# yanconglin/ICP-Flow

Hardware: AMD Instinct MI355X
Metric: cluster-pair ICP registrations/sec (higher is better)
Workload: dtype f32

## Files before the change

### icp_flow_amd/_lib.py

```python
import contextlib
import ctypes
import os
import threading

import torch

_HERE = os.path.dirname(os.path.abspath(__file__))
LIB_PATH = os.environ.get("ICPFLOW_HIP_LIB") or os.path.join(_HERE, "libicpflow_hip.so")

STOP_REFERENCE = 0
STOP_PER_PAIR = 1

if not os.path.exists(LIB_PATH):
    raise ImportError(
        f"{LIB_PATH} not found: build it with `python icp_flow_amd/build.py` "
        "(hipcc --offload-arch=gfx950).  icp_flow_amd has no CPU fallback.")

_L = ctypes.CDLL(LIB_PATH)

_f = ctypes.c_float
_d = ctypes.c_double
_i = ctypes.c_int
_p = ctypes.c_void_p
_sz = ctypes.c_size_t
# ... 33 lines not shown
    "icpflow_cluster_table_pair_workspace_bytes": (_sz, [_i, _i, _i]),
    "icpflow_cluster_table_pair": (_i, [_p, _p, _i, _p, _p, _p, _p, _p, _i, _p, _p, _p, _i, _p, _sz, _p]),
    "icpflow_flow_rigid": (_i, [_p, _p, _i, _p, _p, _i, _p, _p, _p, _sz, _p]),
    "icpflow_flow_rigid_rows": (_i, [_p, _p, _i, _p, _i, _p, _i, _p, _p, _p]),
    "icpflow_dbscan_workspace_bytes": (_sz, [_i]),
    "icpflow_dbscan": (_i, [_p, _i, _p, _i, _d, _i, _p, _p, _p, _p, _sz, _p]),
    "icpflow_hdbscan_mst_workspace_bytes": (_sz, [_i]),
    "icpflow_hdbscan_mst": (_i, [_p, _i, _p, _i, _i, _d, _p, _p, _p, _p, _p, _p, _p, _sz, _p]),
    "icpflow_hdbscan_labels": (_i, [_p, _p, _p, _i, _i, _p]),
    "icpflow_cluster_default_params": (_i, [_p]),
    "icpflow_cluster_pcd_workspace_bytes": (_sz, [_i, _i, _p]),
    "icpflow_cluster_pcd": (_i, [_p, _i, _p, _i, _i, _p, _p, _p, _p, _p, _p, _p, _sz, _p]),
    "icpflow_track_frame_points": (_i, [_p, _p, _i, _p, _p, _i, _p, _p, _p, _p, _p, _p, _p, _p, _p, _p, _p, _p, _sz, _p, _p, _p]),
    "icpflow_ego_default_params": (_i, [_p]),
    "icpflow_ego_state_bytes": (_sz, [_p]),
    "icpflow_ego_create": (_i, [_p, _p, _sz, _p, ctypes.POINTER(_p)]),
    "icpflow_ego_destroy": (_i, [_p]),
    "icpflow_ego_reset": (_i, [_p, _p]),
    "icpflow_ego_register_frame": (_i, [_p, _p, _i, _p, _p]),
    "icpflow_ego_poses": (_i, [_p, _p, _i, ctypes.POINTER(_i)]),
    "icpflow_ego_frame_info": (_i, [_p, _p]),
    "icpflow_ego_downsample": (_i, [_p, _p, _i, _p, _p, _p, _p]),
    "icpflow_ego_register_step": (_i, [_p, _p, _i, _p, _d, _p, _p]),
    "icpflow_ego_map_add": (_i, [_p, _p, _i, _p, _p]),
    "icpflow_ego_map_export": (_i, [_p, _p, _p, _p, _i, _p, _p]),
    "icpflow_egomotion_default_params": (_i, [_p]),
    "icpflow_egomotion_set_params": (_i, [_p, _p]),
    "icpflow_egomotion_deskew": (_i, [_p, _p, _p, _i, _p, _p, _p]),
    "icpflow_egomotion_register_frame_stamped": (_i, [_p, _p, _p, _i, _p, _p, _p]),
    "icpflow_seq_gt_flow_workspace_bytes": (_sz, [_i]),
    "icpflow_seq_gt_flow": (_i, [_p, _p, _p, _i, _p, _i, _p, _i, _i, _p, _p, _p, _sz, _p]),
    "icpflow_seq_metrics_workspace_bytes": (_sz, [_i, _i]),
    "icpflow_seq_metrics": (_i, [_p, _p, _p, _p, _p, _p, _i, _i, _i, _d, _d, _d, _p, _p, _p, _sz, _p]),
    "icpflow_seq_argo_sample": (_i, [_p, _i, _p, _i, _i, _p, _i, _p, _p, _i, _p, _i, _p, _i, _d, _p, _p, _p, _p, _p, _p, _p]),
    "icpflow_seq_class_table_workspace_bytes": (_sz, [_i, _i, _i, _i]),
    "icpflow_seq_class_table": (_i, [_p, _p, _p, _p, _p, _i, _i, _i, _d, _d, _d, _d, _i, _p, _i, _p, _i, _p, _p, _p, _sz, _p]),
    "icpflow_seq_bucket_table_workspace_bytes": (_sz, [_i, _i, _i]),
    "icpflow_seq_bucket_table": (_i, [_p, _p, _p, _p, _p, _i, _i, _i, _d, _d, _d, _d, _i, _p, _i, _p, _p, _p, _sz, _p]),
    "icpflow_seq_segment_table_workspace_bytes": (_sz, [_i, _i]),
    "icpflow_seq_segment_table": (_i, [_p, _p, _i, _p, _p, _d, _p, _i, _p, _p, _sz, _p]),
    "icpflow_ground_default_params": (_i, [_p]),
    "icpflow_ground_workspace_bytes": (_sz, [_i, _p]),
    "icpflow_ground_segment": (_i, [_p, _i, _i, _p, _p, _p, _p, _sz, _p]),
    "icpflow_selftest_vote_quotient": (_i, [_p, _i, _f, _f, _p, _p, _p]),
    "icpflow_selftest_kabsch": (_i, [_p, _p, _i, _i, _p, _p, _p, _p]),
    "icpflow_profile_create": (_i, [_i, ctypes.POINTER(_p)]),
    "icpflow_profile_collect": (_i, [_p, ctypes.POINTER(_d), ctypes.POINTER(_i)]),
    "icpflow_profile_destroy": (_i, [_p]),
}
for _name, (_res, _args) in SIGNATURES.items():
    _fn = getattr(_L, _name)
    _fn.restype = _res
    _fn.argtypes = _args

VERSION = int(_L.icpflow_version())
BUILD_INFO = _L.icpflow_build_info().decode()


def call(name, *args):
    rc = getattr(_L, name)(*args)
    if rc != 0:
        msg = _L.icpflow_last_error()
        raise RuntimeError(f"{name} failed (code {rc}): {msg.decode() if msg else ''}")


GROUND_PATCHES, GROUND_TABLE_COLS = 504, 16
SEQ_MAX_FRAMES = 16
SEG_COLS, SEG_CHUNK_ROWS = 16, 1024
SEQ_OUT_FLOW, SEQ_OUT_POINTS = 0, 1
SEQ_CROP_NONE, SEQ_CROP_XY, SEQ_CROP_XYZ = 0, 1, 2
DTYPE_FLOAT32, DTYPE_FLOAT64 = 0, 1
ARGO_MAX_BACKGROUND = 64
CLASS_MAX_ROWS, CLASS_MAX_BUCKETS, CLASS_MAX_WORDS = 64, 8, 1024
BUCKET_MAX_ROWS, BUCKET_MAX_BUCKETS = 64, 64
SEARCH_AUTO, SEARCH_SCAN, SEARCH_GRID, SEARCH_SWEEP = 0, 1, 2, 3
ARITH_FP64, ARITH_FP32_REFERENCE = 0, 1
OPT_FLAGS = {"no_sorted_vote": 1 << 0, "no_side_stream": 1 << 1, "no_eval_sweep": 1 << 2, "no_check_sweep": 1 << 3,
             "no_score_sweep": 1 << 4, "no_score_prune": 1 << 5, "no_teams": 1 << 6, "no_speculative": 1 << 7,
             "no_adaptive_windows": 1 << 8, "no_persistent": 1 << 9, "no_helpers": 1 << 10,
             "teams_half_gpu": 1 << 11, "no_shared_scans": 1 << 12,
             "no_stage_overlap": 1 << 13, "no_vote_list": 1 << 14, "no_check_reuse": 1 << 15, "no_score_prebound": 1 << 16,
             "two_launch": 1 << 17,
             "no_dir_keys": 1 << 18}


class Options(ctypes.Structure):
    _fields_ = [("struct_size", _sz), ("icp_search", _i), ("icp_arith", _i), ("flags", ctypes.c_uint),
                ("profile", _p), ("d_vote_bins_u32", _p), ("d_icp_init_R", _p), ("d_icp_init_T", _p),
                ("d_icp_history", _p), ("icp_allow_reflection", _i), ("icp_estimate_scale", _i),
                ("d_icp_scale", _p), ("d_icp_init_s", _p), ("d_pair_active", _p)]


class Tables(ctypes.Structure):
    _fields_ = [("d_points_src", _p), ("d_order_src", _p), ("d_table_src", _p), ("d_points_dst", _p), ("d_order_dst", _p),
                ("d_table_dst", _p), ("S", _i), ("D", _i), ("label_stride", _i)]


class Stage(ctypes.Structure):
    _fields_ = [("d_seg", _p), ("d_perm", _p), ("d_si", _p), ("d_di", _p), ("d_clouds", _p), ("d_result", _p), ("K", _i), ("N", _i)]


class Registration(ctypes.Structure):
    _fields_ = [("d_edges_x", _p), ("d_edges_y", _p), ("d_edges_z", _p), ("len_x", _i), ("len_y", _i), ("len_z", _i),
                ("decode_shift", _f), ("thres_dist", _d), ("relative_rmse_thr", _d), ("max_iterations", _i), ("stop_mode", _i)]


class Mt19937(ctypes.Structure):
    _fields_ = [("state", ctypes.c_uint32 * 624), ("index", ctypes.c_int32)]

    @staticmethod
    def from_torch(generator=None):
        raw = (generator if generator is not None else torch.default_generator).get_state().numpy()
        if raw.size < 24 + 8 * 624:
            raise RuntimeError("unexpected layout of torch.Generator.get_state()")
        left = int(raw[8:12].view("<i4")[0])
        nxt = int(raw[16:24].view("<u8")[0])
        mt = Mt19937()
        ctypes.memmove(mt.state, raw[24:24 + 8 * 624].view("<u8").astype("<u4").tobytes(), 4 * 624)
        mt.index = 624 if left == 1 else nxt
        return mt

    def to_torch(self, generator=None):
        import numpy as np
        g = generator if generator is not None else torch.default_generator
        raw = g.get_state().numpy().copy()
        raw[24:24 + 8 * 624] = np.frombuffer(bytes(self.state), dtype="<u4").astype("<u8").view(np.uint8)
        idx = int(self.index)
        raw[8:12] = np.array([1 if idx >= 624 else 625 - idx], "<i4").view(np.uint8)
        raw[16:24] = np.array([idx], "<u8").view(np.uint8)
        g.set_state(torch.from_numpy(raw))


class FrameParams(ctypes.Structure):
    _fields_ = [("struct_size", _sz), ("seed", ctypes.c_uint64), ("generator", _p), ("max_points", _i), ("min_cluster_size", _i),
                ("translation_frame", _f), ("thres_box", _f), ("thres_iou", _f), ("rot_limit_deg", _f), ("thres_error", _f),
                ("tight_padding", _i), ("superset_width", _i)]


CLUSTER_DBSCAN, CLUSTER_HDBSCAN = 0, 1


class ClusterParams(ctypes.Structure):
    _fields_ = [("struct_size", _sz), ("method", _i), ("min_cluster_size", _i), ("num_clusters", _i), ("reserved", _i),
                ("eps", _d), ("cell", _d)]

    @staticmethod
    def defaults(**over):
        p = ClusterParams()
        call("icpflow_cluster_default_params", ctypes.byref(p))
        for k, v in over.items():
            if not hasattr(p, k):
                raise TypeError(f"icpflow_cluster_params_t has no field {k!r}")
            setattr(p, k, v)
        return p


class EgoParams(ctypes.Structure):
    _fields_ = [("struct_size", _sz), ("max_range", _d), ("min_range", _d), ("voxel_size", _d), ("min_motion_th", _d),
                ("initial_threshold", _d), ("convergence", _d), ("max_points_per_voxel", _i), ("max_iterations", _i),
                ("max_points", _i), ("map_capacity", _i)]

    @staticmethod
    def defaults(**over):
        p = EgoParams()
        call("icpflow_ego_default_params", ctypes.byref(p))
        for k, v in over.items():
            if not hasattr(p, k):
                raise TypeError(f"icpflow_ego_params_t has no field {k!r}")
            setattr(p, k, v)
        return p


class EgoMotionParams(ctypes.Structure):
    _fields_ = [("struct_size", _sz), ("deskew", _i), ("reserved", _i), ("mid_stamp", _d), ("fixed_threshold", _d)]

    @staticmethod
    def defaults(**over):
        p = EgoMotionParams()
        call("icpflow_egomotion_default_params", ctypes.byref(p))
        for k, v in over.items():
            if not hasattr(p, k):
                raise TypeError(f"icpflow_ego_motion_params_t has no field {k!r}")
            setattr(p, k, v)
        return p


class GroundParams(ctypes.Structure):
    _fields_ = [("struct_size", _sz), ("sensor_height", _d), ("min_range", _d), ("max_range", _d), ("th_seeds", _d), ("th_dist", _d),
                ("th_seeds_v", _d), ("th_dist_v", _d), ("uprightness_thr", _d), ("adaptive_seed_selection_margin", _d),
                ("num_iter", _i), ("num_lpr", _i), ("num_min_pts", _i), ("num_rings_of_interest", _i),
                ("num_sectors_each_zone", _i * 4), ("num_rings_each_zone", _i * 4)]

    @staticmethod
    def defaults():
        p = GroundParams()
        call("icpflow_ground_default_params", ctypes.byref(p))
        return p


class Profile:

    def __init__(self, capacity):
        self._h = _p()
        call("icpflow_profile_create", int(capacity), ctypes.byref(self._h))

    def collect(self):
        ms, n = _d(0.0), _i(0)
        call("icpflow_profile_collect", self._h, ctypes.byref(ms), ctypes.byref(n))
        return float(ms.value), int(n.value)

    def close(self):
        if self._h:
            _L.icpflow_profile_destroy(self._h)
            self._h = _p()

    __del__ = close


_tls = threading.local()


def _env_default_flags():
    f = 0
    for name, bit in OPT_FLAGS.items():
        if os.environ.get("ICPFLOW_" + name.upper(), "0") not in ("0", ""):
            f |= bit
    return f


_DEFAULT_FLAGS = _env_default_flags()


def _current():
    return getattr(_tls, "stack", None) or [dict(search=0, arith=0, flags=_DEFAULT_FLAGS, profile=None, vote_bins=None,
                                                 icp_init=None, icp_history=None, icp_allow_reflection=False,
                                                 icp_scale=None, pair_active=None)]


@contextlib.contextmanager
def options(search=None, arith=None, profile=None, vote_bins=None, icp_init=None, icp_history=None,
            icp_allow_reflection=None, icp_scale=None, pair_active=None, **switches):
    cur = dict(_current()[-1])
    cur.update(vote_bins=None, icp_init=None, icp_history=None, icp_scale=None, pair_active=None)
    if search is not None:
        cur["search"] = {"auto": 0, "scan": 1, "grid": 2, "sweep": 3}.get(search, search)
    if arith is not None:
        cur["arith"] = {"fp64": 0, "fp32_reference": 1}.get(arith, arith)
    if profile is not None:
        cur["profile"] = profile
    if vote_bins is not None:
        cur["vote_bins"] = vote_bins
    if icp_init is not None:
        cur["icp_init"] = icp_init
    if icp_history is not None:
        cur["icp_history"] = icp_history
    if icp_allow_reflection is not None:
        cur["icp_allow_reflection"] = bool(icp_allow_reflection)
    if icp_scale is not None:
        cur["icp_scale"] = icp_scale
    if pair_active is not None:
        cur["pair_active"] = pair_active
    for k, v in switches.items():
        cur["flags"] = (cur["flags"] | OPT_FLAGS[k]) if v else (cur["flags"] & ~OPT_FLAGS[k])
    stack = getattr(_tls, "stack", None)
    if stack is None:
        stack = _tls.stack = []
    stack.append(cur)
    try:
        yield
    finally:
        stack.pop()


def opt():
    cur = _current()[-1]
    if (cur["search"] == 0 and cur["arith"] == 0 and cur["flags"] == 0 and cur["profile"] is None
            and cur["vote_bins"] is None and cur["icp_init"] is None and cur["icp_history"] is None
            and not cur["icp_allow_reflection"] and cur["icp_scale"] is None and cur.get("pair_active") is None):
        return None
    dp = lambda t: ctypes.c_void_p(t.data_ptr()) if t is not None else None
    o = Options(int(os.environ.get("ICPFLOW_OPTIONS_SIZE", ctypes.sizeof(Options))), int(cur["search"]), int(cur["arith"]), int(cur["flags"]),
                cur["profile"]._h if cur["profile"] is not None else None, dp(cur["vote_bins"]),
                dp(cur["icp_init"][0] if cur["icp_init"] is not None else None),
                dp(cur["icp_init"][1] if cur["icp_init"] is not None else None), dp(cur["icp_history"]),
                1 if cur["icp_allow_reflection"] else 0, 1 if cur["icp_scale"] is not None else 0, dp(cur["icp_scale"]),
                dp(cur["icp_init"][2] if cur["icp_init"] is not None and len(cur["icp_init"]) > 2 else None),
                dp(cur.get("pair_active")))
    _tls.last = o
    return ctypes.cast(ctypes.pointer(o), _p)


def workspace_bytes(B, N, lens=(0, 0, 0)):
    return int(_L.icpflow_workspace_bytes(int(B), int(N), int(lens[0]), int(lens[1]), int(lens[2])))


def require_gpu(*tensors):
    for t in tensors:
        if t is None:
            continue
        if not isinstance(t, torch.Tensor) or not t.is_cuda:
            raise RuntimeError("icp_flow_amd: input must be a GPU (HIP) tensor -- there is no CPU path "
                               "(the reference refuses CPU tensors too, hist_cuda/cpp/hist.cpp:22)")


def cloud(t, name="cloud"):
    require_gpu(t)
    if t.dim() != 3 or t.shape[2] != 4:
        raise RuntimeError(f"{name}: expected shape [B,N,4] (x,y,z,flag), got {tuple(t.shape)}")
    if t.dtype != torch.float32:
        raise RuntimeError(f"{name}: expected float32, got {t.dtype}")
    return t.contiguous()


def ptr(t):
    return ctypes.c_void_p(t.data_ptr()) if t is not None else None


_raw_stream = getattr(torch._C, "_cuda_getCurrentRawStream", None)


def stream_handle(device):
    if _raw_stream is not None:
        idx = device.index if isinstance(device, torch.device) else None
        if idx is None:
            idx = torch.cuda.current_device()
        return int(_raw_stream(idx))
    return int(torch.cuda.current_stream(device).cuda_stream)


def stream(device):
    return ctypes.c_void_p(stream_handle(device))


_ws_cache = {}


def workspace(device, nbytes):
    key = (device.type, device.index, stream_handle(device))
    buf = _ws_cache.get(key)
    if buf is None or buf.numel() < nbytes:
        buf = torch.empty(max(int(nbytes), 1 << 20), dtype=torch.uint8, device=device)
        _ws_cache[key] = buf
    return buf


def workspaces(device, sizes):
# ... 20 lines not shown
```

### icp_flow_amd/build.py

```python
import argparse
import concurrent.futures
import hashlib
import os
import subprocess
import sys

HERE = os.path.dirname(os.path.abspath(__file__))
CSRC = os.path.join(HERE, "csrc")
OBJ = os.path.join(CSRC, "_obj")
OUT = os.path.join(HERE, "libicpflow_hip.so")
SOURCES = ["api.hip", "hist.hip", "nn.hip", "icp.hip", "icp_prep.hip", "icp_plan.hip", "icp_epilogue.hip", "device.hip", "icp_fp32.hip", "pose.hip", "sort.hip", "cluster.hip", "hdbscan.hip", "clusterpcd.hip", "table.hip", "assoc.hip", "frame.hip", "ego.hip", "seqeval.hip", "classeval.hip", "bucketeval.hip", "segeval.hip", "ground.hip",
           "hdbscan_tree.cpp"]
HEADERS = ["common.hpp", "scan.hpp", "kernels.hpp", "kabsch.hpp", "posefuse.hpp", "votekey.hpp", "cluster_util.hpp", "sortdir.hpp", "host.hpp", "carver.hpp", "rowerr.hpp", "clusterpcd_host.hpp", "gridhash.hpp", "icp_instr.hip",
           os.path.join("..", "..", "include", "icpflow_hip.h")]
CFLAGS = ["--offload-arch=gfx950", "-O3", "-std=c++17", "-fPIC", "-ffp-contract=off",
          "-fhip-fp32-correctly-rounded-divide-sqrt", "-Wall", "-Wno-unused-function"]


def hipcc():
    for c in (os.environ.get("HIPCC"), "/opt/rocm/bin/hipcc", "hipcc"):
        if c and (os.path.isabs(c) and os.path.exists(c) or not os.path.isabs(c)):
            return c
    return "hipcc"


def _digest(paths, extra=()):
    h = hashlib.sha256()
    for p in paths:
        h.update(os.path.basename(p).encode())
        with open(p, "rb") as f:
            h.update(f.read())
    for e in extra:
        h.update(str(e).encode())
    return h.hexdigest()


def source_hash():
    return _digest([os.path.join(CSRC, f) for f in SOURCES + HEADERS], CFLAGS)[:16]


_MARK = b"ICPFLOW_SOURCE_HASH="


def built_hash(path=OUT):
    try:
        with open(path, "rb") as f:
            blob = f.read()
    except OSError:
        return None
    k = blob.find(_MARK)
    if k < 0:
        return None
    tag = blob[k + len(_MARK): k + len(_MARK) + 16]
    return tag.decode() if len(tag) == 16 and all(c in b"0123456789abcdef" for c in tag) else None


def stale():
    return built_hash() != source_hash()


def _object(src, extra, objdir):
    hdr = _digest([os.path.join(CSRC, f) for f in HEADERS], CFLAGS + list(extra))
    tag = _digest([os.path.join(CSRC, src)], [hdr])[:16]
    return os.path.join(objdir, f"{os.path.splitext(src)[0]}.{tag}.o")


def _compile(src, obj, argv):
    if not os.path.exists(obj) or "-save-temps=obj" in argv:
        os.makedirs(os.path.dirname(obj), exist_ok=True)
        for old in os.listdir(os.path.dirname(obj)):
            if old.startswith(os.path.splitext(src)[0] + ".") and old.endswith(".o"):
                os.remove(os.path.join(os.path.dirname(obj), old))
        subprocess.check_call(argv, cwd=CSRC)
    return obj


def plan(defines=(), out=None, extra=()):
    out = os.path.abspath(out) if out else OUT
    variant = out != OUT
    if defines and not variant:
        raise ValueError("a build with defines is a variant: give it an `out` of its own (the product library is built as shipped)")
    objdir = os.path.join(OBJ, "variant") if variant else OBJ
    extra = list(extra) + ["-D" + d for d in defines]
    stamp = source_hash()
    compile_, objs = {}, []
    for src in SOURCES:
        e = extra + ([f'-DICPFLOW_SOURCE_HASH="{stamp}"'] if src == "api.hip" else [])
        objs.append(_object(src, e, objdir))
        compile_[src] = [hipcc()] + CFLAGS + e + ["-c", os.path.join(CSRC, src), "-o", objs[-1]]
    return {"compile": compile_, "link": [hipcc(), "--offload-arch=gfx950", "-shared", "-fPIC"] + objs + ["-o", out + ".tmp"], "out": out}


def build(force=False, extra=(), defines=(), out=None, dry_run=False):
    p = plan(defines, out, extra)
    if dry_run:
        return p
# ... 27 lines not shown
```

### icp_flow_amd/csrc/api.hip

```cpp
#include <stdarg.h>
#include <stdio.h>
#include <stdlib.h>
#include <string.h>

#include "kernels.hpp"
#include "posefuse.hpp"
#include "kabsch.hpp"
#include "host.hpp"

using namespace icpflow;

namespace {

thread_local char g_err[512] = "";

}

namespace icpflow {
int report_error(int code, const char *message)
{
    snprintf(g_err, sizeof(g_err), "%s", message);
    return code;
}

// ... 145 lines not shown
        cand = mem.take<float>(b * kCand * 3 * 4);
        {
            size_t qb = (size_t)(scan_qblocks(N, B) > sweep_qblocks(N) ? scan_qblocks(N, B) : sweep_qblocks(N));
            if ((size_t)score_qblocks(N) > qb) qb = (size_t)score_qblocks(N);
            partial = mem.take<double>(b * 12 * qb * kPartial * 8);
            scoreAccum = mem.take<double>(b * 12 * 8);
            ticketScratch = mem.take<int>(256);
            if (shareScratch(B, N)) grid.shareCount = mem.take<int>(b * 12 * kSweepShareSlots * 4);
            accumBytes = align256(b * 12 * 8) + align256(256) + (shareScratch(B, N) ? align256(b * 12 * kSweepShareSlots * 4) : 0);
        }
        Tinit = mem.take<float>(b * 16 * 4);
        M = mem.take<float>(b * 16 * 4);
        state = mem.take<IcpState>(b * sizeof(IcpState));
        ctrl = mem.take<IcpCtrl>(icp_ctrl_bytes(B));
        helpState = mem.take<float>(b * 32 * 4);
        helpOut = mem.take<double>((size_t)kHelpMaxWG * kHelpOutStride * 8);
        grid.H = grid_buckets(N);
        grid.origin = mem.take<float>(b * 4 * 4);
        grid.start = mem.take<int32_t>(b * ((size_t)grid.H + 1) * 4);
        grid.cursor = mem.take<int32_t>(b * (size_t)grid.H * 4);
        grid.pts = mem.take<float>(b * (size_t)N * 16);
        grid.sortX = mem.take<float>(b * (size_t)N * 16);
        grid.sortYsoa = mem.take<float>(b * 3 * (size_t)((N + 15) / 16 * 16) * 4 + 256);
        grid.sortXsoa = mem.take<float>(b * 3 * (size_t)((N + 15) / 16 * 16) * 4 + 256);
        zsortA = mem.take<float>(b * (size_t)N * 16);
        zsortC = mem.take<float>(b * (size_t)N * 16);
        voteKey = mem.take<float>(b * 8 * 4);
        voteWorkCap = vote_work_capacity(B, N);
        if (voteWorkCap != 0) { voteWork = mem.take<int32_t>(voteWorkCap * 4); pairOrder = mem.take<int32_t>(b * 4); }
        if (N > kChunkSortMinN) {
            const size_t cs = b * 2 * (size_t)chunk_sort_length(N) * 4;
            grid.ckey = mem.take<float>(cs);
            grid.cidx = mem.take<int>(cs);
            zckey = mem.take<float>(cs);
            zcidx = mem.take<int>(cs);
            pairBox = mem.take<float>(b * kPairBoxStride * 4);
        }
        grid.axis = mem.take<int32_t>(b * 4);
        grid.scoreList = mem.take<int>(b * 12 * 4);
        if (N <= kMaxSortN) {
            grid.occHdr = mem.take<float>(b * 2 * 8 * 4);
            grid.occBits = mem.take<uint32_t>(b * 2 * (size_t)kOccRings * kOccWords * 4);
            grid.occTot = grid.scoreList;
        }
        if (shareScratch(B, N)) {
            grid.shareBest = mem.take<float>(b * 12 * kSweepShareSlots * 256 * 4);
            if (B <= 32767 && N <= 255 * 256) pairTab = mem.take<int32_t>(b * 4 * 4);
        }
        history = mem.take<float>(b * (size_t)kHistIters * kHistStride * 4);
        team.maxWG = 1024;
        team.wgPair = mem.take<int32_t>((size_t)team.maxWG * 4);
        team.wgRank = mem.take<int32_t>((size_t)team.maxWG * 4);
        team.teamSize = mem.take<int32_t>(b * 4);
        team.next = mem.take<int32_t>(b * 4);
        team.arrived = mem.take<unsigned int>(b * 4);
        team.mom = mem.take<double>((b < 256 ? b : 256) * 2 * (size_t)kMaxTeam * kTeamStride * 8);
        icpSplit = mem.take<int32_t>((b + 64) * 4);
        bytes = mem.total();
    }
};

const GridScratch *search_scratch(Workspace &w, int N, const Opts &o)
{
    int mode = o.search;
    if (o.arith == ICPFLOW_ARITH_FP32_REFERENCE) mode = 1;
    if (mode == 0) mode = (N >= 64 && N <= kMaxSortN) ? 3 : 1;
    if (mode == 3 && N > kMaxSortN) mode = 1;
    if (mode == 1) return nullptr;
    w.grid.mode = mode;
    w.grid.dirKeys = o.on(ICPFLOW_OPT_NO_DIR_KEYS) ? 1 : 0;
    return &w.grid;
}

int parse_options(const char *fn, const icpflow_options_t *opt, Opts &o)
{
    if (opt == nullptr) return 0;
    if (opt->struct_size != sizeof(icpflow_options_t))
        return report_errorf(ICPFLOW_E_ARG, "%s: options struct_size %zu, this library expects %zu", fn, opt->struct_size,
                             sizeof(icpflow_options_t));
    if (opt->icp_search < 0 || opt->icp_search > 3)
        return report_errorf(ICPFLOW_E_ARG, "%s: options.icp_search must be 0..3 (got %d)", fn, opt->icp_search);
    if (opt->icp_arith != ICPFLOW_ARITH_FP64 && opt->icp_arith != ICPFLOW_ARITH_FP32_REFERENCE)
        return report_errorf(ICPFLOW_E_ARG, "%s: options.icp_arith must be 0 or 1 (got %d)", fn, opt->icp_arith);
    if (opt->flags >> 19) return report_errorf(ICPFLOW_E_ARG, "%s: unknown option flags 0x%x", fn, opt->flags);
    o.search = opt->icp_search;
    o.arith = opt->icp_arith;
    o.flags = opt->flags;
    o.profile = reinterpret_cast<LaunchProfile *>(opt->profile);
    o.voteBins = opt->d_vote_bins_u32;
    if ((opt->d_icp_init_R == nullptr) != (opt->d_icp_init_T == nullptr))
        return report_errorf(ICPFLOW_E_ARG, "%s: options.d_icp_init_R and d_icp_init_T come together", fn);
    o.initR = opt->d_icp_init_R;
    o.initT = opt->d_icp_init_T;
    o.history = opt->d_icp_history;
    o.allowReflection = opt->icp_allow_reflection != 0;
    o.estimateScale = opt->icp_estimate_scale != 0;
    o.scaleOut = opt->d_icp_scale;
    o.initS = opt->d_icp_init_s;
    o.pairActive = opt->d_pair_active;
    if (o.initS != nullptr && o.initR == nullptr)
        return report_errorf(ICPFLOW_E_ARG, "%s: options.d_icp_init_s comes with d_icp_init_R / d_icp_init_T", fn);
    return 0;
}

int check_pair_active(const char *fn, const Opts &o, bool fused, int maxIter, int stopMode)
{
    if (o.pairActive == nullptr) return 0;
    if (!fused) return report_errorf(ICPFLOW_E_ARG, "%s: options.d_pair_active is honoured by icpflow_hist_icp / icpflow_hist_icp_eval only", fn);
    if (stopMode != ICPFLOW_STOP_REFERENCE || maxIter < 2 || maxIter > kHistIters || !o.on(ICPFLOW_OPT_NO_SPECULATIVE) ||
        o.arith != ICPFLOW_ARITH_FP64)
        return report_errorf(ICPFLOW_E_ARG, "%s: options.d_pair_active needs the single-launch reference stop (2 <= max_iterations <= %d, "
                                            "fp64 arithmetic, speculation on)", fn, kHistIters);
    return 0;
}

int check_arith(const char *fn, const Opts &o, int maxIter, int stopMode)
{
    if (o.arith != ICPFLOW_ARITH_FP32_REFERENCE) return 0;
    if (stopMode != ICPFLOW_STOP_REFERENCE)
        return report_errorf(ICPFLOW_E_ARG, "%s: ICPFLOW_ARITH_FP32_REFERENCE implements the reference's batch-global stop only", fn);
    if (maxIter > kHistIters)
        return report_errorf(ICPFLOW_E_LIMIT, "%s: ICPFLOW_ARITH_FP32_REFERENCE keeps a per-iteration history: max_iterations <= %d",
                             fn, kHistIters);
    return 0;
}

int check_ws(void *ws, size_t have, size_t need)
{
    if (ws == nullptr || have < need)
        return report_errorf(ICPFLOW_E_WORKSPACE, "workspace too small: have %zu bytes, need %zu", have, need);
    if (((uintptr_t)ws & 15) != 0) return report_errorf(ICPFLOW_E_WORKSPACE, "workspace must be 16-byte aligned");
    return 0;
}

int check_batch(const char *fn, int B, int N)
{
    if (B <= 0 || N <= 0) return report_errorf(ICPFLOW_E_ARG, "%s: B (%d) and N (%d) must be positive", fn, B, N);
    if ((long long)B * N > (1ll << 30)) return report_errorf(ICPFLOW_E_LIMIT, "%s: B*N exceeds 2^30 rows", fn);
    return 0;
}

int check_hist_dims(const char *fn, int lx, int ly, int lz)
{
    if (lx <= 0 || ly <= 0 || lz <= 0)
        return report_errorf(ICPFLOW_E_ARG, "%s: histogram lengths must be positive (%d,%d,%d)", fn, lx, ly, lz);
    if ((long long)lx * ly * lz > (1ll << 28)) return report_errorf(ICPFLOW_E_LIMIT, "%s: histogram too large", fn);
    return 0;
}

struct SideStream {
    hipStream_t stream = nullptr;
    hipEvent_t fork = nullptr, join = nullptr;
    int device = -1;
    bool ok = false;
    void destroy()
    {
        if (stream) (void)hipStreamDestroy(stream);
        if (fork) (void)hipEventDestroy(fork);
        if (join) (void)hipEventDestroy(join);
        stream = nullptr; fork = join = nullptr; ok = false;
    }
    void create()
    {
        ok = hipGetDevice(&device) == hipSuccess &&
             hipStreamCreateWithFlags(&stream, hipStreamNonBlocking) == hipSuccess &&
             hipEventCreateWithFlags(&fork, hipEventDisableTiming) == hipSuccess &&
             hipEventCreateWithFlags(&join, hipEventDisableTiming) == hipSuccess;
// ... 4 lines not shown
{
    constexpr int kSlots = 6;
    struct Slot { SideStream s; hipStream_t caller = nullptr; bool used = false; };
    static thread_local Slot slots[kSlots];
    static thread_local int next = 0;
    static thread_local SideStream none;
    int dev = -1;
    if (hipGetDevice(&dev) != hipSuccess) { none.ok = false; return none; }
    for (int k = 0; k < kSlots; ++k)
        if (slots[k].used && slots[k].caller == caller && slots[k].s.device == dev) return slots[k].s;
    Slot &sl = slots[next];
    next = (next + 1) % kSlots;
    if (!sl.used || sl.s.device != dev) {
        sl.s.destroy();
        sl.s = SideStream{};
        sl.s.create();
    }
    sl.used = true;
    sl.caller = caller;
    return sl.s;
}

struct JoinGuard {
    hipStream_t s = nullptr;
    hipEvent_t join = nullptr;
    ~JoinGuard() { if (join != nullptr) (void)hipStreamWaitEvent(s, join, 0); }
    void joined() { join = nullptr; }
};

int run_icp_and_select(const float *src, const float *dst, Workspace &w, const uint8_t *swap,
                       const float *init, int B, int N, double thres, int maxIter, double relThr,
                       int stopMode, int invertSwapped, float *Tout, int32_t *iters, const Opts &o, hipStream_t s,
                       bool teamPlanned = false, int part = 0, int32_t *pending = nullptr, bool initSumValid = false)
{
    const GridScratch *search = search_scratch(w, N, o);
    const bool sweepCheck = search != nullptr && search->mode == 3 && o.on(ICPFLOW_OPT_NO_CHECK_SWEEP);
    bool historyPending = false;
    IcpOpts io = o.icp(w.grid.sortX);
    io.help = icp_help_carve(w.ctrl, B, w.helpState, w.helpOut);
    io.splitScratch = w.icpSplit;
    io.teamPlanned = teamPlanned;
    if (sweepCheck && o.arith == ICPFLOW_ARITH_FP64) io.historyPending = &historyPending;
    const bool splittable = sweepCheck && o.arith == ICPFLOW_ARITH_FP64 && stopMode == ICPFLOW_STOP_REFERENCE && w.history != nullptr &&
                            o.on(ICPFLOW_OPT_NO_SPECULATIVE) && maxIter > 1 && maxIter <= kHistIters;
    if (part == 1) {
        *pending = 0;
        if (!splittable) return 0;
        if (icp_teams_wanted(&w.team, io, search, B, N, maxIter, stopMode, w.history)) return 0;
        io.pairActive = nullptr;
    }
    if (part == 2 && pending != nullptr && *pending != 0) {
        historyPending = true;
        if (o.pairActive != nullptr) ICPFLOW_TRY(launch_icp_retally(w.ctrl, w.history, o.pairActive, B, maxIter, relThr, s));
    } else {
        ICPFLOW_TRY(launch_icp(src, dst, w.lenA, w.lenC, swap, init, B, N, thres, maxIter, relThr, stopMode,
                               w.state, w.ctrl, search, w.history, &w.team, io, s));
        if (part == 1) {
            if (!historyPending) return report_errorf(ICPFLOW_E_ARG, "icpflow_register_stage_begin: the ICP launch kept no history");
            *pending = 1;
            return 0;
        }
    }
    if (sweepCheck) {
        PoseSource ps{w.state, w.ctrl, historyPending ? w.history : nullptr, init, B, maxIter};
        const double *initSum = (initSumValid && search->presorted && o.on(ICPFLOW_OPT_NO_CHECK_REUSE)) ? w.scoreAccum : nullptr;
        ICPFLOW_TRY(launch_sweep_check(search, src, dst, w.lenA, w.lenC, swap, B, N, init, nullptr, w.partial, s, &ps, o.pairActive,
                                       initSum));
        ICPFLOW_TRY(launch_select(w.partial, sweep_qblocks(N), w.lenA, w.lenC, swap, init, nullptr, B, invertSwapped,
                                  Tout, s, &ps, iters, initSum, o.pairActive));
        return 0;
    }
    ICPFLOW_TRY(launch_compose(w.state, init, B, w.M, s, w.ctrl, iters));
    {
        ICPFLOW_TRY(launch_scan_check(src, dst, w.lenA, w.lenC, swap, B, N, init, w.M, w.partial, s));
        ICPFLOW_TRY(launch_select(w.partial, scan_qblocks(N, B), w.lenA, w.lenC, swap, init, w.M, B,
                                  invertSwapped, Tout, s));
    }
    return 0;
}

int run_init_pose(const float *src, const float *dst, Workspace &w, const uint8_t *swap, int B,
                  int N, const float *ex, int lx, const float *ey, int ly, const float *ez, int lz,
                  float shift, float *Tout, const Opts &o, hipStream_t s, hipEvent_t joinBefore = nullptr,
                  const PairCountFuse *countFuse = nullptr, bool sideBusy = false)
{
    const int lens[3] = {lx, ly, lz};
    if (N <= kMaxSortN && o.on(ICPFLOW_OPT_NO_SORTED_VOTE)) {
        bool planned = false;
        ICPFLOW_TRY(launch_hist_vote_sorted(dst, src, w.lenC, w.lenA, B, N, lens, ex, ey, ez, swap, w.zsortC,
                                            w.zsortA, w.bins, w.zckey, w.zcidx, w.voteKey, s, countFuse, sideBusy,
                                            w.grid.pairBox, o.on(ICPFLOW_OPT_NO_VOTE_LIST) ? w.voteWork : nullptr, w.voteWorkCap,
                                            w.pairOrder, &planned));
        if (planned) w.grid.pairOrder = w.pairOrder;
    } else
        ICPFLOW_TRY(launch_hist_vote(dst, src, B, N, N, nullptr, nullptr, lens, ex, ey, ez, swap, w.bins, s));
    if (o.voteBins != nullptr)
        ICPFLOW_TRY(hipMemcpyAsync(o.voteBins, w.bins, (size_t)B * lx * ly * lz * sizeof(uint32_t),
                                   hipMemcpyDeviceToDevice, s));
    if (w.pairTab != nullptr && B <= 700 && N <= kMaxSortN && o.on(ICPFLOW_OPT_NO_SORTED_VOTE)) {
        ICPFLOW_TRY(launch_sweep_pair_table(w.lenA, w.lenC, swap, w.grid.pairOrder, B, N, w.pairTab, s));
        w.grid.pairTab = w.pairTab;
    }
    PeakDecode dec;
    dec.ex = ex; dec.ey = ey; dec.ez = ez; dec.shift = shift; dec.cand = w.cand;
    ICPFLOW_TRY(launch_hist_peaks_u32(w.bins, B, lx, ly, lz, kTopK, kNmsKernel, w.volA, w.volB,
                                      w.peakVotes, w.peakIdx, s, dec));
    if (score_by_sweep(N, joinBefore != nullptr || w.grid.presorted, o)) {
        if (joinBefore != nullptr) {
            ICPFLOW_TRY(hipStreamWaitEvent(s, joinBefore, 0));
        } else if (!w.grid.presorted) {
            ICPFLOW_TRY(launch_sort_clouds_soa(src, dst, w.lenA, w.lenC, swap, B, N, &w.grid, s));
            w.grid.presorted = 1;
            if (o.on(ICPFLOW_OPT_NO_SCORE_PRUNE) && o.on(ICPFLOW_OPT_NO_SCORE_PREBOUND)) {
                ICPFLOW_TRY(launch_occupancy(&w.grid, B, N, s));
                w.grid.occReady = 1;
            }
        }
        if (o.on(ICPFLOW_OPT_NO_SCORE_PRUNE))
            ICPFLOW_TRY(launch_sweep_score_pruned(&w.grid, w.lenA, w.lenC, swap, B, N, w.cand, w.partial, w.scoreAccum, s));
        else
            ICPFLOW_TRY(launch_sweep_score(&w.grid, w.lenA, w.lenC, swap, B, N, w.cand, w.partial, s));
        ICPFLOW_TRY(launch_score_pick(w.partial, sweep_qblocks(N), w.lenA, w.lenC, swap, w.cand, B, Tout, s, w.scoreAccum));
        w.initSumValid = true;
    } else if (o.on(ICPFLOW_OPT_NO_SCORE_PRUNE)) {
        ICPFLOW_TRY(launch_scan_score_pruned(src, dst, w.lenA, w.lenC, swap, B, N, w.cand, w.partial, w.scoreAccum, s, true));
        ICPFLOW_TRY(launch_score_pick(w.partial, score_qblocks(N), w.lenA, w.lenC, swap, w.cand, B, Tout, s));
    } else {
        ICPFLOW_TRY(launch_scan_score(src, dst, w.lenA, w.lenC, swap, B, N, w.cand, w.partial, s));
        ICPFLOW_TRY(launch_score_pick(w.partial, scan_qblocks(N, B), w.lenA, w.lenC, swap, w.cand, B, Tout, s));
    }
    return 0;
}

}

extern "C" {

int icpflow_version(void) { return ICPFLOW_VERSION; }

#ifndef ICPFLOW_SOURCE_HASH
#define ICPFLOW_SOURCE_HASH "unknown"
#endif
static const char g_build_info[] = "ICPFLOW_SOURCE_HASH=" ICPFLOW_SOURCE_HASH;
const char *icpflow_build_info(void) { return g_build_info + sizeof("ICPFLOW_SOURCE_HASH=") - 1; }

const char *icpflow_last_error(void) { return g_err; }

size_t icpflow_workspace_bytes(int B, int N, int Lx, int Ly, int Lz)
{
    if (B <= 0 || N <= 0) return 0;
    const size_t L = (size_t)(Lx > 0 ? Lx : 0) * (size_t)(Ly > 0 ? Ly : 0) * (size_t)(Lz > 0 ? Lz : 0);
    return Workspace(nullptr, B, N, L).bytes;
}

int icpflow_profile_create(int capacity, icpflow_profile_t **out)
{
    if (out == nullptr) return report_errorf(ICPFLOW_E_ARG, "icpflow_profile_create: null pointer");
    if (capacity < 0 || capacity > (1 << 20)) return report_errorf(ICPFLOW_E_ARG, "icpflow_profile_create: bad capacity %d", capacity);
    hipError_t e = hipSuccess;
    LaunchProfile *p = profile_create(capacity, &e);
    if (p == nullptr) return hip_error(e, "icpflow_profile_create");
    *out = reinterpret_cast<icpflow_profile_t *>(p);
    return 0;
}

int icpflow_profile_collect(icpflow_profile_t *profile, double *total_ms, int *launches)
{
    if (profile == nullptr) return report_errorf(ICPFLOW_E_ARG, "icpflow_profile_collect: null recorder");
    ICPFLOW_TRY(profile_collect(reinterpret_cast<LaunchProfile *>(profile), total_ms, launches));
    return 0;
}

int icpflow_profile_destroy(icpflow_profile_t *profile)
{
    profile_destroy(reinterpret_cast<LaunchProfile *>(profile));
// ... 422 lines not shown
    hipStream_t s = (hipStream_t)stream;
    IcpOpts io = o.icp(w.grid.sortX);
    io.help = icp_help_carve(w.ctrl, B, w.helpState, w.helpOut);
    io.splitScratch = w.icpSplit;
    io.initR = o.initR;
    io.initT = o.initT;
    io.allowReflection = o.allowReflection;
    io.estimateScale = o.estimateScale;
    io.initS = o.initS;
    if ((o.allowReflection || o.estimateScale) && o.arith != ICPFLOW_ARITH_FP64)
        return report_errorf(ICPFLOW_E_ARG, "icpflow_icp: allow_reflection / estimate_scale are not built for ICPFLOW_ARITH_FP32_REFERENCE");
    if (o.history != nullptr &&
        !(stop_mode == ICPFLOW_STOP_REFERENCE && max_iterations > 1 && max_iterations <= kHistIters &&
          o.arith == ICPFLOW_ARITH_FP64 && io.speculative))
        return report_errorf(ICPFLOW_E_ARG, "icpflow_icp: options.d_icp_history needs the single-launch reference stop mode "
                                            "(2 <= max_iterations <= %d, fp64 arithmetic)", kHistIters);
    if (o.initR != nullptr && o.arith != ICPFLOW_ARITH_FP64)
        return report_errorf(ICPFLOW_E_ARG, "icpflow_icp: an initial transform is not built for ICPFLOW_ARITH_FP32_REFERENCE");
    Opts os = o;
    if ((o.estimateScale || o.initS != nullptr) && o.search == 0 && N < 64) os.search = 3;
    const GridScratch *search = search_scratch(w, N, os);
    if ((o.estimateScale || o.initS != nullptr) && (search == nullptr || search->mode != 3))
        return report_errorf(ICPFLOW_E_ARG, "icpflow_icp: estimate_scale / an initial transform with a scale need the sorted-sweep "
                                            "search (the default up to N = %d)", kMaxSortN);
    launch_count_pair(d_X, d_Y, B, N, w.lenA, w.lenC, nullptr, s, w.ctrl, icp_ctrl_bytes(B));
    ICPFLOW_TRY(launch_icp(d_X, d_Y, w.lenA, w.lenC, nullptr, d_pre_pose, B, N, thres, max_iterations,
                           relative_rmse_thr, stop_mode, w.state, w.ctrl, search, w.history, &w.team,
                           io, s));
    if (o.history != nullptr)
        ICPFLOW_TRY(hipMemcpyAsync(o.history, w.history, (size_t)max_iterations * B * kHistStride * sizeof(float),
                                   hipMemcpyDeviceToDevice, s));
    ICPFLOW_TRY(launch_icp_export(w.state, w.ctrl, B, stop_mode, d_R, d_T, d_rmse, d_iters, d_converged, s, o.scaleOut));
    return 0;
}

int icpflow_apply_icp(const float *d_src, const float *d_dst, const float *d_init, int B, int N,
                      double thres_dist, int max_iterations, double relative_rmse_thr, int stop_mode,
                      float *d_T_out, int32_t *d_iters, void *d_ws, size_t ws_bytes,
                      icpflow_stream_t stream, const icpflow_options_t *opt)
{
    Opts o;
    if (int r = parse_options("icpflow_apply_icp", opt, o)) return r;
    if (int r = check_arith("icpflow_apply_icp", o, max_iterations, stop_mode)) return r;
    if (int r = check_pair_active("icpflow_apply_icp", o, false, max_iterations, stop_mode)) return r;
    if (!d_src || !d_dst || !d_init || !d_T_out) return report_errorf(ICPFLOW_E_ARG, "icpflow_apply_icp: null pointer");
    if (int r = check_batch("icpflow_apply_icp", B, N)) return r;
    if (max_iterations <= 0 || max_iterations > kMaxIterCap)
        return report_errorf(ICPFLOW_E_ARG, "icpflow_apply_icp: max_iterations must be in 1..%d", kMaxIterCap);
    if (stop_mode != ICPFLOW_STOP_REFERENCE && stop_mode != ICPFLOW_STOP_PER_PAIR)
        return report_errorf(ICPFLOW_E_ARG, "icpflow_apply_icp: unknown stop_mode %d", stop_mode);
    Workspace w(d_ws, B, N, 0);
    if (int r = check_ws(d_ws, ws_bytes, w.bytes)) return r;
    hipStream_t s = (hipStream_t)stream;
    launch_count_pair(d_src, d_dst, B, N, w.lenA, w.lenC, nullptr, s, w.ctrl, icp_ctrl_bytes(B));
    ICPFLOW_TRY(hipMemcpyAsync(w.Tinit, d_init, (size_t)B * 16 * sizeof(float), hipMemcpyDeviceToDevice, s));
    return run_icp_and_select(d_src, d_dst, w, nullptr, w.Tinit, B, N, thres_dist, max_iterations,
                              relative_rmse_thr, stop_mode, 0, d_T_out, d_iters, o, s);
}

static int hist_icp_core(const float *d_src, const float *d_dst, int B, int N, const float *d_edges_x, int len_x,
                         const float *d_edges_y, int len_y, const float *d_edges_z, int len_z, float decode_shift,
                         double thres_dist, int max_iterations, double relative_rmse_thr, int stop_mode,
                         float *d_T_out, int32_t *d_iters, Workspace &w, const Opts &o, hipStream_t s,
                         int phase = 0, int32_t *carry = nullptr)
{
    if (phase == 2) {
        w.grid.presorted = carry[0];
        w.grid.shareCountClean = 1;
        int32_t pending = carry[2];
        return run_icp_and_select(d_src, d_dst, w, w.swap, w.Tinit, B, N, thres_dist, max_iterations,
                                  relative_rmse_thr, stop_mode, 1, d_T_out, d_iters, o, s, carry[1] != 0, 2, &pending, carry[3] != 0);
    }
    const bool countInSort = N <= kMaxSortN && N <= kChunkSortMinN && o.on(ICPFLOW_OPT_NO_SORTED_VOTE);
    if (!countInSort) {
        launch_count_pair(d_src, d_dst, B, N, w.lenA, w.lenC, w.swap, s, w.ctrl, icp_ctrl_bytes(B), w.scoreAccum,
                          w.accumBytes, w.pairBox);
        w.grid.pairBox = w.pairBox;
    }
    hipEvent_t join = nullptr;
    bool teamPlanned = false;
    JoinGuard guard;
    const GridScratch *search = search_scratch(w, N, o);
    SideStream *side = nullptr;
    if (search != nullptr && search->mode == 3 && N >= 64 && o.on(ICPFLOW_OPT_NO_SIDE_STREAM)) {
        side = &side_stream(s);
        if (!side->ok) side = nullptr;
    }
    if (side != nullptr) {
        ICPFLOW_TRY(hipEventRecord(side->fork, s));
        ICPFLOW_TRY(hipStreamWaitEvent(side->stream, side->fork, 0));
        const bool wantOcc = score_by_sweep(N, true, o) && o.on(ICPFLOW_OPT_NO_SCORE_PRUNE) && o.on(ICPFLOW_OPT_NO_SCORE_PREBOUND);
        const bool occFirst = wantOcc && N <= kChunkSortMinN;
        hipError_t se = hipSuccess;
        if (occFirst) {
            se = launch_occupancy_raw(d_src, d_dst, w.lenA, w.lenC, w.swap, B, N, &w.grid, countInSort ? 2 : 0, side->stream);
            if (se == hipSuccess) w.grid.occReady = 1;
        }
        if (se == hipSuccess)
            se = launch_sort_clouds_soa(d_src, d_dst, w.lenA, w.lenC, w.swap, B, N, &w.grid, side->stream, countInSort ? 2 : 0);
        if (se == hipSuccess && wantOcc && !occFirst) {
            se = launch_occupancy(&w.grid, B, N, side->stream);
            if (se == hipSuccess) w.grid.occReady = 1;
        }
        if (se == hipSuccess && !countInSort && phase != 1 &&
            icp_teams_wanted(&w.team, o.icp(w.grid.sortX), search, B, N, max_iterations, stop_mode, w.history)) {
            launch_icp_team_plan(&w.team, w.lenA, w.lenC, w.swap, B, N, o.icp(w.grid.sortX), side->stream);
            teamPlanned = true;
        }
        const hipError_t je = hipEventRecord(side->join, side->stream);
        if (je == hipSuccess) { guard.s = s; guard.join = side->join; }
        ICPFLOW_TRY(se);
        ICPFLOW_TRY(je);
        w.grid.presorted = 1;
        join = side->join;
    }
    PairCountFuse fuse{};
    if (countInSort) {
        fuse.swapOut = w.swap;
        fuse.zero0 = w.ctrl; fuse.bytes0 = icp_ctrl_bytes(B);
        fuse.zero1 = w.scoreAccum; fuse.bytes1 = w.accumBytes;
    }
    w.grid.shareCountClean = 1;
    w.grid.sweepTicket = w.ticketScratch;
    const bool sweepScore = score_by_sweep(N, join != nullptr, o);
    if (int r = run_init_pose(d_src, d_dst, w, w.swap, B, N, d_edges_x, len_x, d_edges_y, len_y, d_edges_z,
                              len_z, decode_shift, w.Tinit, o, s, sweepScore ? join : nullptr,
                              countInSort ? &fuse : nullptr, join != nullptr))
        return r;
    if (join != nullptr && !sweepScore) ICPFLOW_TRY(hipStreamWaitEvent(s, join, 0));
    guard.joined();
    if (phase == 1) {
        carry[0] = w.grid.presorted;
        carry[1] = teamPlanned ? 1 : 0;
        carry[3] = w.initSumValid ? 1 : 0;
        return run_icp_and_select(d_src, d_dst, w, w.swap, w.Tinit, B, N, thres_dist, max_iterations, relative_rmse_thr,
                                  stop_mode, 1, d_T_out, d_iters, o, s, teamPlanned, 1, &carry[2]);
    }
    return run_icp_and_select(d_src, d_dst, w, w.swap, w.Tinit, B, N, thres_dist, max_iterations,
                              relative_rmse_thr, stop_mode, 1, d_T_out, d_iters, o, s, teamPlanned, 0, nullptr, w.initSumValid);
}

int icpflow_hist_icp(const float *d_src, const float *d_dst, int B, int N, const float *d_edges_x,
                     int len_x, const float *d_edges_y, int len_y, const float *d_edges_z, int len_z,
                     float decode_shift, double thres_dist, int max_iterations, double relative_rmse_thr,
                     int stop_mode, float *d_T_out, int32_t *d_iters, void *d_ws, size_t ws_bytes,
                     icpflow_stream_t stream, const icpflow_options_t *opt)
{
    Opts o;
    if (int r = parse_options("icpflow_hist_icp", opt, o)) return r;
    if (int r = check_arith("icpflow_hist_icp", o, max_iterations, stop_mode)) return r;
    if (int r = check_pair_active("icpflow_hist_icp", o, true, max_iterations, stop_mode)) return r;
    if (!d_src || !d_dst || !d_edges_x || !d_edges_y || !d_edges_z || !d_T_out)
        return report_errorf(ICPFLOW_E_ARG, "icpflow_hist_icp: null pointer");
    if (int r = check_batch("icpflow_hist_icp", B, N)) return r;
    if (int r = check_hist_dims("icpflow_hist_icp", len_x, len_y, len_z)) return r;
    if (max_iterations <= 0 || max_iterations > kMaxIterCap)
        return report_errorf(ICPFLOW_E_ARG, "icpflow_hist_icp: max_iterations must be in 1..%d", kMaxIterCap);
    if (stop_mode != ICPFLOW_STOP_REFERENCE && stop_mode != ICPFLOW_STOP_PER_PAIR)
        return report_errorf(ICPFLOW_E_ARG, "icpflow_hist_icp: unknown stop_mode %d", stop_mode);
    const size_t L = (size_t)len_x * len_y * len_z;
    if (L < (size_t)kTopK) return report_errorf(ICPFLOW_E_ARG, "icpflow_hist_icp: fewer than 5 bins");
    Workspace w(d_ws, B, N, L);
    if (int r = check_ws(d_ws, ws_bytes, w.bytes)) return r;
    return hist_icp_core(d_src, d_dst, B, N, d_edges_x, len_x, d_edges_y, len_y, d_edges_z, len_z, decode_shift,
                         thres_dist, max_iterations, relative_rmse_thr, stop_mode, d_T_out, d_iters, w, o,
                         (hipStream_t)stream);
}

int icpflow_hist_icp_many(int K, const float *const *d_src, const float *const *d_dst, const int *B, int N,
                          const float *d_edges_x, int len_x, const float *d_edges_y, int len_y,
                          const float *d_edges_z, int len_z, float decode_shift, double thres_dist,
                          int max_iterations, double relative_rmse_thr, int stop_mode, float *const *d_T_out,
                          int32_t *const *d_iters, void *const *d_ws, const size_t *ws_bytes,
                          icpflow_stream_t stream, const icpflow_options_t *opt)
{
    if (K <= 0 || K > 64) return report_errorf(ICPFLOW_E_ARG, "icpflow_hist_icp_many: K must be in 1..64 (got %d)", K);
    if (!d_src || !d_dst || !B || !d_T_out || !d_iters || !d_ws || !ws_bytes)
        return report_errorf(ICPFLOW_E_ARG, "icpflow_hist_icp_many: null pointer");
    for (int k = 0; k < K; ++k)
        for (int j = 0; j < k; ++j)
            if (d_ws[k] == d_ws[j]) return report_errorf(ICPFLOW_E_WORKSPACE, "icpflow_hist_icp_many: batches %d and %d share a workspace", j, k);
    hipStream_t s = (hipStream_t)stream;
    constexpr int kWorkers = 4;
    struct Pool {
        hipStream_t w[kWorkers] = {nullptr, nullptr, nullptr, nullptr};
        hipEvent_t fork = nullptr, join[kWorkers] = {nullptr, nullptr, nullptr, nullptr};
        int device = -1;
        bool ok = false;
    };
    static thread_local Pool pool;
    int dev = -1;
    ICPFLOW_TRY(hipGetDevice(&dev));
    if (!pool.ok || pool.device != dev) {
        pool = Pool{};
        pool.device = dev;
        ICPFLOW_TRY(hipEventCreateWithFlags(&pool.fork, hipEventDisableTiming));
        for (int k = 0; k < kWorkers; ++k) {
            ICPFLOW_TRY(hipStreamCreateWithFlags(&pool.w[k], hipStreamNonBlocking));
            ICPFLOW_TRY(hipEventCreateWithFlags(&pool.join[k], hipEventDisableTiming));
        }
        pool.ok = true;
    }
    const int used = K < kWorkers ? K : kWorkers;
    ICPFLOW_TRY(hipEventRecord(pool.fork, s));
    for (int k = 0; k < used; ++k) ICPFLOW_TRY(hipStreamWaitEvent(pool.w[k], pool.fork, 0));
    int rc = 0;
    for (int k = 0; k < K && rc == 0; ++k)
        rc = icpflow_hist_icp(d_src[k], d_dst[k], B[k], N, d_edges_x, len_x, d_edges_y, len_y, d_edges_z, len_z, decode_shift,
                              thres_dist, max_iterations, relative_rmse_thr, stop_mode, d_T_out[k], d_iters[k], d_ws[k],
                              ws_bytes[k], pool.w[k % kWorkers], opt);
// ... 133 lines not shown
```

### icp_flow_amd/csrc/hist.hip

```cpp
#include "common.hpp"
#include "kernels.hpp"
#include "votekey.hpp"

namespace icpflow {

__global__ __launch_bounds__(256) void count_valid_kernel(const float4 *__restrict__ pts, int N,
                                                          int32_t *__restrict__ len)
{
    __shared__ int scratch[4];
    const int b = blockIdx.x;
    const float4 *p = pts + (size_t)b * N;
    int c[1] = {0};
    for (int i = threadIdx.x; i < N; i += blockDim.x) c[0] += (p[i].w > 0.0f) ? 1 : 0;
    block_sum<1, int>(c, scratch);
    if (threadIdx.x == 0) len[b] = c[0];
}

__global__ __launch_bounds__(1024) void count_pair_kernel(const float4 *__restrict__ A, const float4 *__restrict__ C,
                                                         int N, int32_t *__restrict__ lenA,
                                                         int32_t *__restrict__ lenC, uint8_t *__restrict__ swap,
                                                         uint32_t *__restrict__ zero0, unsigned words0,
                                                         uint32_t *__restrict__ zero1, unsigned words1,
                                                         float *__restrict__ boxes)
{
    __shared__ int scratch[2 * 16];
    const int b = blockIdx.x;
    for (unsigned k = blockIdx.x * blockDim.x + threadIdx.x; k < words0; k += gridDim.x * blockDim.x) zero0[k] = 0u;
    for (unsigned k = blockIdx.x * blockDim.x + threadIdx.x; k < words1; k += gridDim.x * blockDim.x) zero1[k] = 0u;
    const float4 *pa = A + (size_t)b * N, *pc = C + (size_t)b * N;
    int c[2] = {0, 0};
    for (int i0 = threadIdx.x; i0 < N; i0 += 4 * blockDim.x) {
        float wa[4], wc[4];
#pragma unroll
        for (int u = 0; u < 4; ++u) {
            const int i = min(i0 + u * (int)blockDim.x, N - 1);
            wa[u] = pa[i].w; wc[u] = pc[i].w;
        }
#pragma unroll
        for (int u = 0; u < 4; ++u)
            if (i0 + u * (int)blockDim.x < N) { c[0] += (wa[u] > 0.0f) ? 1 : 0; c[1] += (wc[u] > 0.0f) ? 1 : 0; }
    }
    block_sum<2, int>(c, scratch);
    if (threadIdx.x == 0) {
        lenA[b] = c[0];
        lenC[b] = c[1];
        if (swap != nullptr) swap[b] = c[0] > c[1] ? 1 : 0;
    }
    if (boxes == nullptr) return;
    __shared__ float boxSh[16][kPairBoxStride];
    float bx[kPairBoxStride];
#pragma unroll
    for (int k = 0; k < kPairBoxStride; ++k) bx[k] = ((k % 6) < 3) ? kInf : -kInf;
#pragma unroll
    for (int side = 0; side < 2; ++side) {
        const float4 *pts = side == 0 ? pa : pc;
        const int n = c[side];
        for (int j0 = threadIdx.x; j0 < n; j0 += 4 * blockDim.x) {
            float4 q[4];
#pragma unroll
            for (int u = 0; u < 4; ++u) q[u] = pts[min(j0 + u * (int)blockDim.x, n - 1)];
#pragma unroll
            for (int u = 0; u < 4; ++u) {
                if (j0 + u * (int)blockDim.x >= n) continue;
                const float v[3] = {q[u].x, q[u].y, q[u].z};
#pragma unroll
                for (int k = 0; k < 3; ++k) {
                    bx[side * 12 + 6 + k] = fminf(bx[side * 12 + 6 + k], v[k]);
                    bx[side * 12 + 9 + k] = fmaxf(bx[side * 12 + 9 + k], v[k]);
                    if (q[u].w > 0.0f) {
                        bx[side * 12 + k] = fminf(bx[side * 12 + k], v[k]);
                        bx[side * 12 + 3 + k] = fmaxf(bx[side * 12 + 3 + k], v[k]);
                    }
                }
            }
        }
    }
#pragma unroll
    for (int k = 0; k < kPairBoxStride; ++k)
#pragma unroll
        for (int o = kWave / 2; o > 0; o >>= 1) {
            const float other = __shfl_xor(bx[k], o, kWave);
            bx[k] = ((k % 6) < 3) ? fminf(bx[k], other) : fmaxf(bx[k], other);
        }
    if ((threadIdx.x & (kWave - 1)) == 0)
#pragma unroll
// ... 203 lines not shown

constexpr int kZsortBlock = 1024;

struct ZsortCount {
    int32_t *lenP, *lenQ;
    uint8_t *swap;
    uint32_t *zero0; unsigned words0;
    uint32_t *zero1; unsigned words1;
};

__global__ __launch_bounds__(kZsortBlock) void zsort_kernel(const float4 *__restrict__ P,
                                                           const float4 *__restrict__ Qc,
                                                           const int32_t *__restrict__ nP,
                                                           const int32_t *__restrict__ nQ, int N, int NP2full,
                                                           float4 *__restrict__ Ps, float4 *__restrict__ Qs,
                                                           uint32_t *__restrict__ bins, int L,
                                                           const float *__restrict__ ez, int len_z,
                                                           float *__restrict__ keyRec, ZsortCount cnt)
{
    extern __shared__ __attribute__((aligned(16))) unsigned char dynLds[];
    unsigned long long *kv = reinterpret_cast<unsigned long long *>(dynLds);
    __shared__ float bbScratch[6 * (kZsortBlock / kWave)];
    __shared__ float keyShared[kVoteKeyStride];
    const int b = blockIdx.x;
    int cntP, cntQ;
    if (cnt.lenP != nullptr) {
        const unsigned stride = gridDim.x * gridDim.y * kZsortBlock;
        const unsigned first = (blockIdx.y * gridDim.x + blockIdx.x) * kZsortBlock + threadIdx.x;
        for (unsigned k = first; k < cnt.words0; k += stride) cnt.zero0[k] = 0u;
        for (unsigned k = first; k < cnt.words1; k += stride) cnt.zero1[k] = 0u;
        __shared__ int cntScratch[2 * (kZsortBlock / kWave)];
        const float4 *pp = P + (size_t)b * N, *pq = Qc + (size_t)b * N;
        int c[2] = {0, 0};
        for (int i = threadIdx.x; i < N; i += kZsortBlock) {
            c[0] += (pp[i].w > 0.0f) ? 1 : 0;
            c[1] += (pq[i].w > 0.0f) ? 1 : 0;
        }
        block_sum<2, int>(c, cntScratch);
        cntP = c[0]; cntQ = c[1];
        if (blockIdx.y == 0 && threadIdx.x == 0) {
            cnt.lenP[b] = cntP;
            cnt.lenQ[b] = cntQ;
            if (cnt.swap != nullptr) cnt.swap[b] = cntQ > cntP ? 1 : 0;
        }
    } else {
        cntP = nP[b]; cntQ = nQ[b];
    }
    const float4 *in = (blockIdx.y == 0 ? P : Qc) + (size_t)b * N;
    float4 *out = (blockIdx.y == 0 ? Ps : Qs) + (size_t)b * N;
    {
        const int half = (L + 1) / 2;
        uint32_t *h = bins + (size_t)b * L + (size_t)blockIdx.y * half;
        const int cnt = blockIdx.y == 0 ? half : L - half;
        for (int k = threadIdx.x; k < cnt; k += kZsortBlock) h[k] = 0u;
    }
    const int n = min(blockIdx.y == 0 ? cntP : cntQ, N);
    const VoteKey vk = vote_key_params(P + (size_t)b * N, min(cntP, N), Qc + (size_t)b * N, min(cntQ, N),
                                       ez[len_z - 1] - ez[0], bbScratch, keyShared);
    if (blockIdx.y == 0 && threadIdx.x < kVoteKeyStride) keyRec[(size_t)b * kVoteKeyStride + threadIdx.x] = keyShared[threadIdx.x];
    int NP2 = kWave;
    while (NP2 < n) NP2 <<= 1;
    NP2 = min(NP2, NP2full);
    for (int j = threadIdx.x; j < NP2; j += kZsortBlock) {
        float k = kInf;
        if (j < n) {
            const float4 q = in[j];
            if (q.w > 0.0f) k = vote_key(vk, q.x, q.y, q.z);
        }
        kv[j] = sort_pack(k, j);
    }
    __syncthreads();
    bitonic_sort_lds(kv, NP2);
    for (int r = threadIdx.x; r < N; r += kZsortBlock) {
        float4 o = make_float4(0.f, 0.f, kInf, kInf);
        if (r < NP2) {
            const unsigned long long w = kv[r];
            const float k = sort_key_of(w);
            if (k < kInf) { o = in[sort_index_of(w)]; o.w = k; }
        }
        out[r] = o;
    }
}

template <int BLOCK, int SPLIT = 1>
__global__ __launch_bounds__(BLOCK) void hist_vote_sorted_kernel(
    const float4 *__restrict__ Xs, const float4 *__restrict__ Ys, const int32_t *__restrict__ nXv,
    const int32_t *__restrict__ nYv, int N, int len_x, int len_y, int len_z,
    const float *__restrict__ ex, const float *__restrict__ ey, const float *__restrict__ ez,
    const uint8_t *__restrict__ swap, int useLds, uint32_t *__restrict__ bins_u32,
    const float *__restrict__ keyRec, int span, const int32_t *__restrict__ work, int nPairs)
{
    extern __shared__ __attribute__((aligned(16))) unsigned char smem[];
    float4 *tile = reinterpret_cast<float4 *>(smem);
    uint32_t *lhist = reinterpret_cast<uint32_t *>(smem + sizeof(float4) * kVoteTile);
    int item = 0;
    if (work != nullptr) {
        item = work[blockIdx.x];
        if (item < 0) return;
    }
    const int b = work != nullptr ? (item & 1023) : (int)blockIdx.y;
    const VoteKey vk = vote_key_load(keyRec + (size_t)b * kVoteKeyStride);
    const bool sw = swap != nullptr && swap[b] != 0;
    const float4 *xb = (sw ? Ys : Xs) + (size_t)b * N;
    const float4 *yb = (sw ? Xs : Ys) + (size_t)b * N;
    const int nx = (sw ? nYv : nXv)[b], ny = (sw ? nXv : nYv)[b];
    const int tsplit = (N + span - 1) / span;
    constexpr int kRows = BLOCK / SPLIT;
    constexpr int kRowWaves = kRows / kWave;
    const int rowBlocks = work != nullptr ? (nx + kRows - 1) / kRows : (N + kRows - 1) / kRows;
    const int rb = work != nullptr ? ((item >> 10) & 255) : (int)blockIdx.x / tsplit;
    const int jBegin = (work != nullptr ? (item >> 18) : (int)blockIdx.x % tsplit) * span;
    if (rb * kWave >= nx || jBegin >= ny) return;
    const float min_x = ex[0], max_x = ex[len_x - 1];
    const float min_y = ey[0], max_y = ey[len_y - 1];
    const float min_z = ez[0], max_z = ez[len_z - 1];
    const int L = len_x * len_y * len_z;
    uint32_t *gb = bins_u32 + (size_t)b * L;
    const bool lastPair = b + 1 == nPairs;
    const int Lx = L + vote_overflow_bins(len_y, len_z);
    const int limit = lastPair ? L : 0x7fffffff;
    const int lane = threadIdx.x & (kWave - 1);
    const int wv = (int)(threadIdx.x >> 6);
    const int share = SPLIT > 1 ? wv / kRowWaves : 0;
    const int i = ((SPLIT > 1 ? wv % kRowWaves : wv) * rowBlocks + rb) * kWave + lane;
    const bool xvalid = i < nx;
    float4 xi = make_float4(0.f, 0.f, 0.f, 0.f);
    if (xvalid) xi = xb[i];
    if (useLds) {
        for (int k = threadIdx.x; k < Lx; k += BLOCK) lhist[k] = 0u;
    }
    const AxisQuot dqx = axis_quot_make(min_x, max_x), dqy = axis_quot_make(min_y, max_y), dqz = axis_quot_make(min_z, max_z);
    const bool allFast = dqx.fast && dqy.fast && dqz.fast && (long long)len_x * len_y < (1 << 23) && len_z < (1 << 23);
    const VoteBox box{min_x, min_y, min_z, max_x, max_y, max_z, len_x, len_y, len_z};
    float zlo = xvalid ? xi.z : kInf, zhi = xvalid ? xi.z : -kInf;
#pragma unroll
    for (int o = kWave / 2; o > 0; o >>= 1) {
        zlo = fminf(zlo, __shfl_xor(zlo, o, kWave));
        zhi = fmaxf(zhi, __shfl_xor(zhi, o, kWave));
    }
    const float slack = 1e-3f * (fabsf(max_z) + fabsf(min_z)) + 1e-5f * (fabsf(zlo) + fabsf(zhi)) + 1e-6f;
    const float wlo = zlo - max_z - slack, whi = zhi - min_z + slack;
    float ulo = kInf, uhi = -kInf;
    int slabLo = 0, slabHi = 0;
    if (vk.wide) {
        const float xu = vk.uaxis == 0 ? xi.x : xi.y;
        ulo = xvalid ? xu : kInf; uhi = xvalid ? xu : -kInf;
#pragma unroll
        for (int o = kWave / 2; o > 0; o >>= 1) {
            ulo = fminf(ulo, __shfl_xor(ulo, o, kWave));
            uhi = fmaxf(uhi, __shfl_xor(uhi, o, kWave));
        }
        const float minu = vk.uaxis == 0 ? min_x : min_y, maxu = vk.uaxis == 0 ? max_x : max_y;
        const float su = 0.0625f + 1e-5f * (fabsf(ulo) + fabsf(uhi) + fabsf(vk.u0));
        ulo = ulo - maxu - vk.u0 - su;
        uhi = uhi - minu - vk.u0 + su;
        slabLo = (int)floorf((wlo - vk.z0) / vk.h);
        slabHi = (int)floorf((whi - vk.z0) / vk.h);
    }
    const int jEnd = min(ny, jBegin + span);
    for (int j0 = jBegin; j0 < jEnd; j0 += kVoteTile) {
        const int tn = min(kVoteTile, jEnd - j0);
        __syncthreads();
        for (int k = threadIdx.x; k < tn; k += BLOCK) tile[k] = yb[j0 + k];
        __syncthreads();
        if (!(zlo <= zhi)) continue;
        const float *zkey = reinterpret_cast<const float *>(tile) + 3;
        const int nwin = vk.wide ? max(slabHi - slabLo + 1, 0) : 1;
        for (int win = 0; win < nwin; ++win) {
        int r0, r1;
        if (vk.wide) {
            const float sbase = (float)(slabLo + win) * kSlabStride;
            const float klo = sbase + fmaxf(ulo, 0.f), khi = sbase + fminf(uhi, kSlabStride - 0.5f);
            if (!(klo <= khi)) continue;
            r0 = sorted_count_below<false>(zkey, 4, tn, klo, lane);
            r1 = sorted_count_below<true>(zkey, 4, tn, khi, lane);
        } else {
            r0 = sorted_count_below<false>(zkey, 4, tn, wlo, lane);
            r1 = sorted_count_below<true>(zkey, 4, tn, whi, lane);
        }
        if (!xvalid) continue;
        r0 = __builtin_amdgcn_readfirstlane(r0);
        r1 = __builtin_amdgcn_readfirstlane(r1);
        if (SPLIT > 1) {
            const int len = max(r1 - r0, 0);
            r1 = r0 + (len * (share + 1)) / SPLIT;
            r0 = r0 + (len * share) / SPLIT;
        }
#ifdef ICPFLOW_VOTE_STATS
        if (r1 > r0) {
            const unsigned long long rows = __ballot(true);
            if (lane == __builtin_ctzll(rows)) {
                atomicAdd(&g_vote_stats[0], (unsigned long long)(r1 - r0) * __popcll(rows));
                atomicAdd(&g_vote_stats[2], (unsigned long long)(r1 - r0));
                atomicAdd(&g_vote_stats[3], 1ull);
            }
        }
#endif
        if (allFast && dqx.pow2 && dqy.pow2) {
            if (useLds) vote_range<true, true, true>(tile, r0, r1, xi, box, dqx, dqy, dqz, lhist, limit);
            else vote_range<true, false, true>(tile, r0, r1, xi, box, dqx, dqy, dqz, gb, limit);
        } else if (allFast) {
            if (useLds) vote_range<true, true>(tile, r0, r1, xi, box, dqx, dqy, dqz, lhist, limit);
            else vote_range<true, false>(tile, r0, r1, xi, box, dqx, dqy, dqz, gb, limit);
        } else {
            if (useLds) vote_range<false, true>(tile, r0, r1, xi, box, dqx, dqy, dqz, lhist, limit);
            else vote_range<false, false>(tile, r0, r1, xi, box, dqx, dqy, dqz, gb, limit);
        }
        }
    }
    if (useLds) {
        __syncthreads();
        for (int k = threadIdx.x; k < (lastPair ? L : Lx); k += BLOCK) {
            const uint32_t v = lhist[k];
            if (v) atomicAdd(&gb[k], v);
        }
    }
}

__global__ __launch_bounds__(1024) void vote_plan_kernel(const int32_t *__restrict__ nXv, const int32_t *__restrict__ nYv,
                                                         const uint8_t *__restrict__ swap, int nPairs, int rows, int span,
                                                         int U, int32_t *__restrict__ work, int32_t *__restrict__ orderOut)
{
    __shared__ int wk[1024], by_[1024], order[1024], start[1025], part[16];
    const int t = threadIdx.x, lane = t & (kWave - 1), wv = t >> 6;
    int mine = 0, byMine = 0;
    if (t < nPairs) {
        const bool sw = swap != nullptr && swap[t] != 0;
        const int nx = (sw ? nYv : nXv)[t], ny = (sw ? nXv : nYv)[t];
        byMine = (ny + span - 1) / span;
        mine = ((nx + rows - 1) / rows) * byMine;
    }
    wk[t] = mine;
    __syncthreads();
    int rank = 0;
    if (t < nPairs)
        for (int u = 0; u < nPairs; ++u) { const int o = wk[u]; rank += (o > mine || (o == mine && u < t)) ? 1 : 0; }
    __syncthreads();
    if (t < nPairs) { order[rank] = t; by_[rank] = byMine; }
    if (blockIdx.x == 0 && t < nPairs && orderOut != nullptr) orderOut[rank] = t;
    __syncthreads();
    const int v = t < nPairs ? wk[order[t]] : 0;
    int inc = v;
#pragma unroll
    for (int o = 1; o < kWave; o <<= 1) { const int up = __shfl_up(inc, o, kWave); if (lane >= o) inc += up; }
    if (lane == kWave - 1) part[wv] = inc;
    __syncthreads();
    int base = 0;
    for (int k = 0; k < wv; ++k) base += part[k];
    start[t] = base + inc - v;
    if (t == 1023) start[1024] = base + inc;
    __syncthreads();
    const int total = start[1024];
    const int e = blockIdx.x * 1024 + t;
    if (e >= U) return;
    int item = -1;
    if (e < total) {
        int lo = 0, hi = nPairs;
        while (hi - lo > 1) { const int mid = (lo + hi) >> 1; if (start[mid] <= e) lo = mid; else hi = mid; }
        const int q = e - start[lo], by = by_[lo];
        item = order[lo] | ((q / by) << 10) | ((q % by) << 18);
    }
    work[e] = item;
}

size_t vote_work_capacity(int B, int N)
{
    if (N <= 1023 || B > 1024) return 0;
    const size_t full = (size_t)B * ((N + 127) / 128) * ((N + 511) / 512);
    return full > 32768 ? full : 32768;
}

hipError_t launch_hist_vote_sorted(const float *X, const float *Y, int32_t *nX, int32_t *nY,
                                   int B, int N, const int lens[3], const float *ex, const float *ey,
                                   const float *ez, const uint8_t *swap, float *sortX, float *sortY,
                                   uint32_t *bins_u32, float *ckey, int *cidx, float *keyRec, hipStream_t s,
                                   const PairCountFuse *fuse, bool sideBusy, const float *boxes, int32_t *work, size_t workCap,
                                   int32_t *orderOut, bool *planned)
{
    if (planned != nullptr) *planned = false;
    if (fuse != nullptr && N > kChunkSortMinN) return hipErrorInvalidValue;
    const size_t L = (size_t)lens[0] * lens[1] * lens[2];
    int NP2 = 64;
    while (NP2 < N) NP2 <<= 1;
    if ((size_t)NP2 * 8 > 64 * 1024) {
        static std::atomic<unsigned long long> attr{0ull};
        ensure_dynamic_lds(reinterpret_cast<const void *>(&zsort_kernel), 128 * 1024, &attr);
    }
    if (N > kChunkSortMinN && ckey != nullptr) {
        hipError_t e = launch_zsort_chunked(X, Y, nX, nY, B, N, sortX, sortY, bins_u32, (int)L, ckey, cidx, ez, lens[2],
                                            keyRec, s, boxes);
        if (e != hipSuccess) return e;
    } else {
        ZsortCount zc{};
        if (fuse != nullptr) {
            zc.lenP = nX; zc.lenQ = nY; zc.swap = fuse->swapOut;
            zc.zero0 = (uint32_t *)fuse->zero0; zc.words0 = (unsigned)(fuse->bytes0 / 4);
            zc.zero1 = (uint32_t *)fuse->zero1; zc.words1 = (unsigned)(fuse->bytes1 / 4);
        }
        hipLaunchKernelGGL(zsort_kernel, dim3(B, 2), dim3(kZsortBlock), (size_t)NP2 * 8, s, (const float4 *)X,
                           (const float4 *)Y, nX, nY, N, NP2, (float4 *)sortX, (float4 *)sortY, bins_u32, (int)L, ez,
                           lens[2], keyRec, zc);
    }
    const size_t tile_bytes = sizeof(float4) * kVoteTile;
    const size_t lds_hist = tile_bytes + sizeof(uint32_t) * (L + (size_t)vote_overflow_bins(lens[1], lens[2]));
    const int useLds = lds_hist <= 64 * 1024;
#ifndef ICPFLOW_VOTE_WIDE_N
#define ICPFLOW_VOTE_WIDE_N 1023
#endif
#ifndef ICPFLOW_VOTE_LIST_MIN_N
#define ICPFLOW_VOTE_LIST_MIN_N 4097
#endif
#ifndef ICPFLOW_VOTE_LIST_SPAN
#define ICPFLOW_VOTE_LIST_SPAN 2048
#endif
    constexpr int kVoteListSpan = ICPFLOW_VOTE_LIST_SPAN;
#ifndef ICPFLOW_VOTE_WIDE_B
#define ICPFLOW_VOTE_WIDE_B 2
#endif
    constexpr int kVoteWideB = ICPFLOW_VOTE_WIDE_B;
    constexpr int kVoteWideN = ICPFLOW_VOTE_WIDE_N;
    const int cus = device_cus();
    const long long wgs256 = (long long)((N + kVoteBlock - 1) / kVoteBlock) * ((N + kVoteSpan * kVoteTile - 1) / (kVoteSpan * kVoteTile)) * B;
    int block = wgs256 >= 4LL * cus ? 512 : kVoteBlock;
    int span = kVoteSpan * kVoteTile;
    const long long waves = (long long)((N + kWave - 1) / kWave) * B;
    if (waves < 8LL * cus) {
        block = 1024;
        while (span > 256 && waves * ((N + span - 1) / span) < 32LL * cus) span >>= 1;
    }
    const int tsplit = (N + span - 1) / span;
    const bool split = useLds && !sideBusy && block != 1024 && wgs256 >= 2LL * cus && wgs256 <= 4LL * cus;
    if (useLds && N > kVoteWideN && B <= kVoteWideB * cus) {
        dim3 grid(((N + 127) / 128) * tsplit, B);
        const int lspan = (work != nullptr && N >= ICPFLOW_VOTE_LIST_MIN_N) ? min(span, kVoteListSpan) : span;
        const int ltsplit = (N + lspan - 1) / lspan;
        const size_t U = (size_t)((N + 127) / 128) * ltsplit * B;
        const bool listed = work != nullptr && U <= workCap && B <= 1024 && (N + 127) / 128 <= 256 && ltsplit <= 128 &&
                            N >= ICPFLOW_VOTE_LIST_MIN_N;
        if (listed) {
            hipLaunchKernelGGL(vote_plan_kernel, dim3((unsigned)((U + 1023) / 1024)), dim3(1024), 0, s, nX, nY, swap, B, 128, lspan,
                               (int)U, work, orderOut);
            if (planned != nullptr) *planned = orderOut != nullptr;
            grid = dim3((unsigned)U, 1);
        }
        hipLaunchKernelGGL((hist_vote_sorted_kernel<512, 4>), grid, dim3(512), lds_hist, s,
                           (const float4 *)sortX, (const float4 *)sortY, nX, nY, N, lens[0], lens[1], lens[2], ex, ey,
                           ez, swap, useLds, bins_u32, keyRec, listed ? lspan : span, listed ? work : (const int32_t *)nullptr, B);
        return hipGetLastError();
    }
    if (block == 1024) {
        dim3 grid(((N + 1023) / 1024) * tsplit, B);
        hipLaunchKernelGGL(hist_vote_sorted_kernel<1024>, grid, dim3(1024), useLds ? lds_hist : tile_bytes, s,
                           (const float4 *)sortX, (const float4 *)sortY, nX, nY, N, lens[0], lens[1], lens[2], ex, ey,
                           ez, swap, useLds, bins_u32, keyRec, span, (const int32_t *)nullptr, B);
    } else if (block == 512 && !split) {
        dim3 grid(((N + 511) / 512) * tsplit, B);
        hipLaunchKernelGGL(hist_vote_sorted_kernel<512>, grid, dim3(512), useLds ? lds_hist : tile_bytes, s,
                           (const float4 *)sortX, (const float4 *)sortY, nX, nY, N, lens[0], lens[1], lens[2], ex, ey,
                           ez, swap, useLds, bins_u32, keyRec, span, (const int32_t *)nullptr, B);
    } else if (split) {
        dim3 grid(((N + kVoteBlock - 1) / kVoteBlock) * tsplit, B);
        hipLaunchKernelGGL((hist_vote_sorted_kernel<2 * kVoteBlock, 2>), grid, dim3(2 * kVoteBlock), lds_hist, s,
                           (const float4 *)sortX, (const float4 *)sortY, nX, nY, N, lens[0], lens[1], lens[2], ex, ey,
                           ez, swap, useLds, bins_u32, keyRec, span, (const int32_t *)nullptr, B);
    } else {
        dim3 grid(((N + kVoteBlock - 1) / kVoteBlock) * tsplit, B);
        hipLaunchKernelGGL(hist_vote_sorted_kernel<kVoteBlock>, grid, dim3(kVoteBlock), useLds ? lds_hist : tile_bytes, s,
                           (const float4 *)sortX, (const float4 *)sortY, nX, nY, N, lens[0], lens[1], lens[2], ex, ey,
                           ez, swap, useLds, bins_u32, keyRec, span, (const int32_t *)nullptr, B);
    }
    return hipGetLastError();
}

__global__ void u32_to_f32_kernel(const uint32_t *__restrict__ in, float *__restrict__ out, size_t n)
{
    const size_t i = (size_t)blockIdx.x * blockDim.x + threadIdx.x;
    if (i < n) out[i] = (float)in[i];
}

hipError_t launch_hist_vote(const float *X, const float *Y, int B, int NX, int NY,
                            const float mins[3], const float maxs[3], const int lens[3],
                            const float *ex, const float *ey, const float *ez,
                            const uint8_t *swap, uint32_t *bins_u32, hipStream_t s)
{
    VoteBox box{mins ? mins[0] : 0.f, mins ? mins[1] : 0.f, mins ? mins[2] : 0.f,
                maxs ? maxs[0] : 0.f, maxs ? maxs[1] : 0.f, maxs ? maxs[2] : 0.f,
                lens[0], lens[1], lens[2]};
    const size_t L = (size_t)lens[0] * lens[1] * lens[2];
    hipError_t e = hipMemsetAsync(bins_u32, 0, sizeof(uint32_t) * L * (size_t)B, s);
    if (e != hipSuccess) return e;
    const int rows = swap ? (NX > NY ? NX : NY) : NX;
    dim3 grid((rows + kVoteBlock - 1) / kVoteBlock, B);
    const size_t tile_bytes = sizeof(float4) * kVoteTile;
    const size_t lds_hist = tile_bytes + sizeof(uint32_t) * (L + (size_t)vote_overflow_bins(lens[1], lens[2]));
    if (lds_hist <= 64 * 1024) {
        hipLaunchKernelGGL(hist_vote_kernel<true>, grid, dim3(kVoteBlock), lds_hist, s,
                           (const float4 *)X, (const float4 *)Y, NX, NY, box, ex, ey, ez, swap,
                           bins_u32);
    } else {
        hipLaunchKernelGGL(hist_vote_kernel<false>, grid, dim3(kVoteBlock), tile_bytes, s,
                           (const float4 *)X, (const float4 *)Y, NX, NY, box, ex, ey, ez, swap,
                           bins_u32);
    }
    return hipGetLastError();
}

hipError_t launch_u32_to_f32(const uint32_t *in, float *out, size_t n, hipStream_t s)
{
    hipLaunchKernelGGL(u32_to_f32_kernel, dim3((unsigned)((n + 255) / 256)), dim3(256), 0, s, in, out, n);
    return hipGetLastError();
}

constexpr int kPeakBlock = 1024;
constexpr int kPeakMaxK = 8;
constexpr int kPeakList = 512;
#ifndef ICPFLOW_PEAK_PARTS
#define ICPFLOW_PEAK_PARTS 7
#endif

template <int R>
__device__ __forceinline__ uint32_t peak_window_max(const uint32_t *__restrict__ V, int f, int c, int n, int stride)
{
    uint32_t v[2 * R + 1];
#pragma unroll
    for (int dq = -R; dq <= R; ++dq) v[dq + R] = V[f + (min(max(c + dq, 0), n - 1) - c) * stride];
    uint32_t m = v[0];
// ... 303 lines not shown
```

### icp_flow_amd/csrc/icp_prep.hip

```cpp
#include "scan.hpp"
#include "sortdir.hpp"
#include "kernels.hpp"
#include "gridhash.hpp"

namespace icpflow {

constexpr int kGridBlock = 256;

int grid_buckets(int N)
{
    int H = 64;
    while (H < 2 * N) H <<= 1;
    return H;
}

__global__ __launch_bounds__(kGridBlock) void grid_build_kernel(
    const float *__restrict__ X, const float *__restrict__ Y, const int32_t *__restrict__ lenX,
    const int32_t *__restrict__ lenY, const uint8_t *__restrict__ swap, int N, int H, float invh,
    float *__restrict__ origin, int32_t *__restrict__ start, int32_t *__restrict__ cursor,
    float4 *__restrict__ pts)
{
    __shared__ int part[kGridBlock];
    const int b = blockIdx.x, tid = threadIdx.x;
    const bool sw = swap != nullptr && swap[b] != 0;
    const float4 *yb = reinterpret_cast<const float4 *>(sw ? X : Y) + (size_t)b * N;
    const int n = (sw ? lenX : lenY)[b];
    int32_t *st = start + (size_t)b * (H + 1);
    int32_t *cu = cursor + (size_t)b * H;
    float4 *out = pts + (size_t)b * N;
    const unsigned mask = (unsigned)H - 1u;
    float4 o4 = make_float4(0.f, 0.f, 0.f, 0.f);
    if (n > 0) o4 = yb[0];
    if (tid == 0) { origin[b * 4 + 0] = o4.x; origin[b * 4 + 1] = o4.y; origin[b * 4 + 2] = o4.z; origin[b * 4 + 3] = 0.f; }
    for (int k = tid; k <= H; k += kGridBlock) st[k] = 0;
    __syncthreads();
    for (int j = tid; j < n; j += kGridBlock) {
        const float4 q = yb[j];
        const unsigned h = grid_hash(grid_cell(q.x, o4.x, invh), grid_cell(q.y, o4.y, invh),
                                     grid_cell(q.z, o4.z, invh), mask);
        atomicAdd(&st[h + 1], 1);
    }
    __syncthreads();
    const int per = (H + kGridBlock - 1) / kGridBlock;
    const int lo = 1 + tid * per, hi = min(1 + (tid + 1) * per, H + 1);
    int sum = 0;
    for (int k = lo; k < hi; ++k) sum += st[k];
    part[tid] = sum;
    __syncthreads();
    if (tid == 0) {
        int run = 0;
        for (int k = 0; k < kGridBlock; ++k) { const int v = part[k]; part[k] = run; run += v; }
    }
    __syncthreads();
    int run = part[tid];
    for (int k = lo; k < hi; ++k) { run += st[k]; st[k] = run; }
    __syncthreads();
    for (int k = tid; k < H; k += kGridBlock) cu[k] = st[k];
    __syncthreads();
    for (int j = tid; j < n; j += kGridBlock) {
        const float4 q = yb[j];
        const unsigned h = grid_hash(grid_cell(q.x, o4.x, invh), grid_cell(q.y, o4.y, invh),
                                     grid_cell(q.z, o4.z, invh), mask);
        const int pos = atomicAdd(&cu[h], 1);
        out[pos] = make_float4(q.x, q.y, q.z, __int_as_float(j));
    }
}

void launch_grid_build(const float *X, const float *Y, const int32_t *lenX, const int32_t *lenY, const uint8_t *swap, int B,
                       int N, float invh, const GridScratch *grid, hipStream_t s)
{
    hipLaunchKernelGGL(grid_build_kernel, dim3(B), dim3(kGridBlock), 0, s, X, Y, lenX, lenY, swap, N,
                       grid->H, invh, grid->origin, grid->start, grid->cursor, (float4 *)grid->pts);
}

constexpr int kSortBlock = 1024;
static std::atomic<unsigned long long> g_sortAttr{0ull};

__global__ __launch_bounds__(kSortBlock) void sort_clouds_kernel(
    const float *__restrict__ X, const float *__restrict__ Y, const int32_t *__restrict__ lenX,
    const int32_t *__restrict__ lenY, const uint8_t *__restrict__ swap, const float *__restrict__ prePose,
    int N, int NP2, int32_t *__restrict__ axisOut, float4 *__restrict__ Xs, float4 *__restrict__ Ys,
    float *__restrict__ Ysoa, float *__restrict__ Xsoa, int selfCount, int dirKeys)
{
    extern __shared__ __attribute__((aligned(16))) unsigned char dynLds[];
    unsigned long long *kv = reinterpret_cast<unsigned long long *>(dynLds);
    __shared__ float bb[6 * (kSortBlock / kWave)];
    __shared__ int axisSh;
    const int b = blockIdx.x, tid = threadIdx.x;
    const bool moving = blockIdx.y == 1;
    int cX, cY;
    bool sw;
    if (selfCount) {
        __shared__ int cntScratch[2 * (kSortBlock / kWave)];
        const float4 *px = reinterpret_cast<const float4 *>(X) + (size_t)b * N;
        const float4 *py = reinterpret_cast<const float4 *>(Y) + (size_t)b * N;
        int c[2] = {0, 0};
        for (int i = tid; i < N; i += kSortBlock) {
            c[0] += (px[i].w > 0.0f) ? 1 : 0;
            c[1] += (py[i].w > 0.0f) ? 1 : 0;
        }
        block_sum<2, int>(c, cntScratch);
        cX = c[0]; cY = c[1];
        sw = selfCount == 2 && cX > cY;
    } else {
        cX = lenX[b]; cY = lenY[b];
        sw = swap != nullptr && swap[b] != 0;
    }
    const float4 *xb = reinterpret_cast<const float4 *>(sw ? Y : X) + (size_t)b * N;
    const float4 *yb = reinterpret_cast<const float4 *>(sw ? X : Y) + (size_t)b * N;
    const int nx = sw ? cY : cX, ny = sw ? cX : cY;
    float mn[3] = {kInf, kInf, kInf}, mx[3] = {-kInf, -kInf, -kInf};
    for (int j = tid; j < ny; j += kSortBlock) {
        const float4 q = yb[j];
        mn[0] = fminf(mn[0], q.x); mn[1] = fminf(mn[1], q.y); mn[2] = fminf(mn[2], q.z);
        mx[0] = fmaxf(mx[0], q.x); mx[1] = fmaxf(mx[1], q.y); mx[2] = fmaxf(mx[2], q.z);
    }
#pragma unroll
    for (int k = 0; k < 3; ++k)
#pragma unroll
        for (int o = kWave / 2; o > 0; o >>= 1) {
            mn[k] = fminf(mn[k], __shfl_xor(mn[k], o, kWave));
            mx[k] = fmaxf(mx[k], __shfl_xor(mx[k], o, kWave));
        }
    if ((tid & (kWave - 1)) == 0) {
#pragma unroll
        for (int k = 0; k < 3; ++k) { bb[(tid >> 6) * 6 + k] = mn[k]; bb[(tid >> 6) * 6 + 3 + k] = mx[k]; }
    }
    __syncthreads();
    __shared__ float boxSh[6];
    if (tid == 0) {
        float e[3];
        for (int k = 0; k < 3; ++k) {
            float lo = bb[k], hi = bb[3 + k];
            for (int w = 1; w < kSortBlock / kWave; ++w) { lo = fminf(lo, bb[w * 6 + k]); hi = fmaxf(hi, bb[w * 6 + 3 + k]); }
            e[k] = hi - lo;
            boxSh[k] = lo; boxSh[3 + k] = hi;
        }
        const int a = (e[0] >= e[1] && e[0] >= e[2]) ? 0 : (e[1] >= e[2] ? 1 : 2);
        axisSh = a;
    }
    __syncthreads();
    if (dirKeys && ny >= kSortDirMinN && nx >= kSortDirMinMoving) {
        __shared__ unsigned int scoreSh[kSortCodes];
        (void)choose_sort_code<kSortBlock>(yb, ny, boxSh, axisSh, reinterpret_cast<unsigned int *>(dynLds), scoreSh, &axisSh);
    }
    if (tid == 0 && !moving) axisOut[b] = axisSh;
    const int axis = axisSh;
    float dirX = 0.f, dirY = 0.f;
    if (axis >= 3) sort_dir(axis, dirX, dirY);
    const int n = moving ? nx : ny;
    const float4 *cloud = moving ? xb : yb;
    PointXf pre;
    pre.kind = (moving && prePose) ? XF_AFFINE : XF_NONE;
    pre.a = (moving && prePose) ? affine_from_pose(prePose + (size_t)b * 16) : affine_identity();
    int np2 = kWave;
    while (np2 < n) np2 <<= 1;
    np2 = min(np2, NP2);
    for (int j = tid; j < np2; j += kSortBlock) {
        float k = kInf;
        if (j < n) {
            const float4 q = cloud[j];
            float px, py, pz;
            xf_apply(pre, q.x, q.y, q.z, px, py, pz);
            k = sort_key_of(axis, dirX, dirY, px, py, pz);
        }
        kv[j] = sort_pack(k, j);
    }
    __syncthreads();
    bitonic_sort_lds(kv, np2);
    float4 *out = (moving ? Xs : Ys) + (size_t)b * N;
    const int NP16 = (N + kChunk - 1) / kChunk * kChunk;
    float *soa = moving ? (Xsoa ? Xsoa + (size_t)b * 3 * NP16 : nullptr) : Ysoa + (size_t)b * 3 * NP16;
    for (int r = tid; r < (soa ? NP16 : n); r += kSortBlock) {
        float px = kInf, py = kInf, pz = kInf;
        if (r < n) {
            const int j = sort_index_of(kv[r]);
            const float4 q = cloud[j];
            xf_apply(pre, q.x, q.y, q.z, px, py, pz);
            out[r] = make_float4(px, py, pz, __int_as_float(j));
        }
        if (soa) { soa[r] = px; soa[NP16 + r] = py; soa[2 * NP16 + r] = pz; }
    }
}

static bool sort_is_chunked(int N, const GridScratch *grid) { return N > kChunkSortMinN && grid->ckey != nullptr; }

hipError_t launch_sort_clouds(const float *X, const float *Y, const int32_t *lenX, const int32_t *lenY, const uint8_t *swap,
                              const float *prePose, int B, int N, const GridScratch *grid, bool wantXsoa, const float *boxes,
                              int selfCount, hipStream_t s)
{
    if (selfCount != 0 && N > kChunkSortMinN) return hipErrorInvalidValue;
    float *Xsoa = wantXsoa ? grid->sortXsoa : nullptr;
    int NP2 = 64;
    while (NP2 < N) NP2 <<= 1;
    if ((size_t)NP2 * 8 > 64 * 1024)
        ensure_dynamic_lds(reinterpret_cast<const void *>(&sort_clouds_kernel), 128 * 1024, &g_sortAttr);
    if (sort_is_chunked(N, grid))
        return launch_sort_clouds_chunked(X, Y, lenX, lenY, swap, prePose, B, N, grid->axis, grid->sortX, grid->pts,
                                          grid->sortYsoa, Xsoa, grid->ckey, grid->cidx, s, boxes, grid->dirKeys);
    hipLaunchKernelGGL(sort_clouds_kernel, dim3(B, 2), dim3(kSortBlock), (size_t)NP2 * 8, s, X, Y, lenX, lenY, swap,
                       prePose, N, NP2, grid->axis, (float4 *)grid->sortX, (float4 *)grid->pts, grid->sortYsoa, Xsoa,
                       selfCount, grid->dirKeys);
    return hipSuccess;
}

hipError_t launch_sort_clouds_soa(const float *X, const float *Y, const int32_t *lenX, const int32_t *lenY,
                                  const uint8_t *swap, int B, int N, const GridScratch *grid, hipStream_t s, int selfCount)
{
    const hipError_t e = launch_sort_clouds(X, Y, lenX, lenY, swap, nullptr, B, N, grid, true, grid->pairBox, selfCount, s);
    return (e != hipSuccess || sort_is_chunked(N, grid)) ? e : hipGetLastError();
}

}
```

### icp_flow_amd/csrc/kernels.hpp

```cpp
#pragma once
#include <hip/hip_runtime.h>
#include <atomic>
#include <stddef.h>
#include <stdint.h>

#include "../../include/icpflow_hip.h"

namespace icpflow {

constexpr int ICPFLOW_STOP_REFERENCE_ = ICPFLOW_STOP_REFERENCE;
constexpr int ICPFLOW_STOP_PER_PAIR_ = ICPFLOW_STOP_PER_PAIR;

constexpr int kPartial = 8;
constexpr int kMaxIterCap = 1024;
constexpr int kCand = 6;
constexpr int kTopK = 5;
constexpr int kNmsKernel = 11;

struct IcpState {
    float R[9];
    float T[3];
    float rmse;
    int active;
    int iters;
    float s;
};

struct IcpCtrl {
    int done;
    int iters;
    int error;
    int ticket;
    int finished;
    int pad[3];
    int notconv[kMaxIterCap];
    unsigned long long tally[kMaxIterCap];
};

struct HelpPair {
    int iter;
    int nclaim;
    int epoch;
    int passes;
    int from[4];
    int pad[8];
};
constexpr int kHelpSlots = 3;
constexpr int kHelpMaxEpoch = 255;
constexpr int kHelpMaxWG = 1024;
constexpr int kHelpOutStride = 16 * 18;
struct IcpHelp {
    HelpPair *pair = nullptr;
    int *tag = nullptr;
    int *owner = nullptr;
    float *state = nullptr;
    double *out = nullptr;
};
inline size_t icp_ctrl_bytes(int B);

#ifndef ICPFLOW_MAX_TEAM
#define ICPFLOW_MAX_TEAM 16
#endif
constexpr int kMaxTeam = ICPFLOW_MAX_TEAM;
constexpr int kTeamStride = 20;
constexpr int kShareParts = 8;
struct IcpTeam {
    int32_t *wgPair;
    int32_t *wgRank;
    int32_t *teamSize;
    int32_t *next;
    unsigned int *arrived;
    double *mom;
    int maxWG;
};

inline size_t icp_ctrl_bytes(int B)
{
    return sizeof(IcpCtrl) + (size_t)B * sizeof(HelpPair) + 2 * (size_t)kHelpMaxWG * sizeof(int);
}
inline IcpHelp icp_help_carve(IcpCtrl *ctrl, int B, float *state, double *out)
{
    IcpHelp h;
    h.pair = reinterpret_cast<HelpPair *>(ctrl + 1);
    h.tag = reinterpret_cast<int *>(h.pair + B);
    h.owner = h.tag + kHelpMaxWG;
    h.state = state;
    h.out = out;
    return h;
}

constexpr int kHistIters = 128;
constexpr int kHistStride = 16;

void launch_count_valid(const float *pts, int B, int N, int32_t *len, hipStream_t s);
void launch_count_pair(const float *A, const float *C, int B, int N, int32_t *lenA, int32_t *lenC, uint8_t *swap,
                       hipStream_t s, void *zero0 = nullptr, size_t bytes0 = 0, void *zero1 = nullptr, size_t bytes1 = 0,
                       float *boxes = nullptr);
hipError_t launch_hist_vote(const float *X, const float *Y, int B, int NX, int NY,
                            const float mins[3], const float maxs[3], const int lens[3],
                            const float *ex, const float *ey, const float *ez,
                            const uint8_t *swap, uint32_t *bins_u32, hipStream_t s);
struct PairCountFuse {
    uint8_t *swapOut;
    void *zero0; size_t bytes0;
    void *zero1; size_t bytes1;
};
hipError_t launch_hist_vote_sorted(const float *X, const float *Y, int32_t *nX, int32_t *nY,
                                   int B, int N, const int lens[3], const float *ex, const float *ey,
                                   const float *ez, const uint8_t *swap, float *sortX, float *sortY,
                                   uint32_t *bins_u32, float *ckey, int *cidx, float *keyRec, hipStream_t s,
                                   const PairCountFuse *fuse = nullptr, bool sideBusy = false, const float *boxes = nullptr,
                                   int32_t *work = nullptr, size_t workCap = 0, int32_t *orderOut = nullptr, bool *planned = nullptr);
size_t vote_work_capacity(int B, int N);
constexpr int kChunkSortMinN = 4096;
constexpr int kPairBoxStride = 24;
int chunk_sort_length(int N);
hipError_t launch_zsort_chunked(const float *P, const float *Q, const int32_t *nP, const int32_t *nQ, int B, int N,
                                float *outP, float *outQ, uint32_t *bins, int L, float *ckey, int *cidx,
                                const float *ez, int len_z, float *keyRec, hipStream_t s, const float *boxes = nullptr);
hipError_t launch_sort_clouds_chunked(const float *X, const float *Y, const int32_t *lenX, const int32_t *lenY,
                                      const uint8_t *swap, const float *prePose, int B, int N, int32_t *axisOut,
                                      float *Xs, float *Ys, float *Ysoa, float *Xsoa, float *ckey, int *cidx,
                                      hipStream_t s, const float *boxes = nullptr, int dirKeys = 0);
hipError_t launch_u32_to_f32(const uint32_t *in, float *out, size_t n, hipStream_t s);
hipError_t launch_hist_peaks_f32(const float *bins, int B, int Lx, int Ly, int Lz, int k,
                                 int kernel_size, uint32_t *wsA, uint32_t *wsB, float *votes,
                                 int64_t *idx, hipStream_t s);
struct PeakDecode {
    const float *ex = nullptr, *ey = nullptr, *ez = nullptr;
    float shift = 0.f;
    float *cand = nullptr;
};
hipError_t launch_hist_peaks_u32(const uint32_t *bins, int B, int Lx, int Ly, int Lz, int k,
                                 int kernel_size, uint32_t *wsA, uint32_t *wsB, float *votes,
                                 int64_t *idx, hipStream_t s, PeakDecode dec = PeakDecode{});

struct GridScratch;
hipError_t launch_sweep_pair_table(const int32_t *lenA, const int32_t *lenC, const uint8_t *swap, const int32_t *pairOrder,
                                   int B, int N, int32_t *tab, hipStream_t s);
int scan_qblocks(int maxRows, int batch);
int sweep_qblocks(int maxRows);
hipError_t launch_sweep_eval(const GridScratch *grid, const int32_t *len1, const int32_t *len2, int B, int N,
                             const float *pose, float thres, float *srcT, double *partial, hipStream_t s, const uint8_t *swap = nullptr,
                             const uint8_t *active = nullptr);
struct PoseSource;
hipError_t launch_sweep_check(const GridScratch *grid, const float *X, const float *Y, const int32_t *lenA,
                              const int32_t *lenC, const uint8_t *swap, int B, int N, const float *poseInit,
                              const float *poseFinal, double *partial, hipStream_t s, const PoseSource *fused = nullptr,
                              const uint8_t *active = nullptr, const double *initSum = nullptr);
hipError_t launch_occupancy(const GridScratch *grid, int B, int N, hipStream_t s);
hipError_t launch_occupancy_raw(const float *X, const float *Y, const int32_t *lenX, const int32_t *lenY, const uint8_t *swap, int B, int N,
                                const GridScratch *grid, int selfCount, hipStream_t s);
hipError_t launch_sweep_score(const GridScratch *grid, const int32_t *lenA, const int32_t *lenC, const uint8_t *swap,
                              int B, int N, const float *cand, double *partial, hipStream_t s);
hipError_t launch_sweep_score_pruned(const GridScratch *grid, const int32_t *lenA, const int32_t *lenC,
                                     const uint8_t *swap, int B, int N, const float *cand, double *partial,
                                     double *accum, hipStream_t s);
hipError_t launch_scan_score(const float *A, const float *C, const int32_t *lenA, const int32_t *lenC,
                             const uint8_t *swap, int B, int N, const float *cand, double *partial,
                             hipStream_t s);
int score_qblocks(int maxRows);
hipError_t launch_scan_score_pruned(const float *A, const float *C, const int32_t *lenA, const int32_t *lenC,
                                    const uint8_t *swap, int B, int N, const float *cand, double *partial,
                                    double *accum, hipStream_t s, bool accumCleared = false);
hipError_t launch_scan_check(const float *A, const float *C, const int32_t *lenA, const int32_t *lenC,
                             const uint8_t *swap, int B, int N, const float *poseInit,
                             const float *poseFinal, double *partial, hipStream_t s);
hipError_t launch_scan_eval(const float *A, const float *C, const int32_t *lenA, const int32_t *lenC,
                            int B, int N, const float *pose, float thres, double *partial, hipStream_t s);
hipError_t launch_scan_nn(const float *Qp, const float *Tp, int B, int NQ, int NT, int strideQ,
                          int strideT, const int32_t *lenQ, const int32_t *lenT, int sqrt_dist,
                          int64_t *idx, float *dist, hipStream_t s);

constexpr int kOccWords = 1024;
#ifndef ICPFLOW_OCC_RINGS
#define ICPFLOW_OCC_RINGS 3
#endif
constexpr int kOccRings = ICPFLOW_OCC_RINGS;
constexpr int kSweepShareSlots = 16;
struct GridScratch {
    int mode;
    int H;
    float *origin;
    int32_t *start;
    int32_t *cursor;
    float *pts;
    float *sortX;
    float *sortYsoa;
    float *sortXsoa;
    int32_t *axis;
    int dirKeys;
    float *ckey;
    int *cidx;
    const float *pairBox;
    const int32_t *pairTab;
// ... 144 lines not shown
```

### icp_flow_amd/csrc/nn.hip

```cpp
#include "scan.hpp"
#include "sortdir.hpp"
#include "kernels.hpp"
#include "posefuse.hpp"

namespace icpflow {

enum ScanMode : int { MODE_SCORE = 0, MODE_CHECK = 1, MODE_EVAL = 2, MODE_NN = 3 };

struct ScanParams {
    const float *A;
    const float *C;
    const int32_t *lenA;
    const int32_t *lenC;
    const uint8_t *swap;
    int N;
    int NT;
    int strideQ, strideT;
    int njobs;
    int qblocks;
    const float *cand;
    int subBegin, subCount, prune;
    double *accum;
    int split;
    const float *poseA;
    const float *poseB;
    float thres;
    double *partial;
    int64_t *idx;
    float *dist;
    int sqrt_dist;
};

template <int Q, int MODE>
__global__ __launch_bounds__(kScanBlock) void nn_scan_kernel(ScanParams p)
{
    __shared__ ScanTile tileMem;
    ScanTile *tile = &tileMem;
    __shared__ double red[(kScanBlock / kWave) * kPartial];

    const int lin = blockIdx.x;
    int job = (lin / (8 * p.qblocks)) * 8 + (lin & 7);
    int qb = (lin >> 3) % p.qblocks;
    if (MODE == MODE_SCORE && p.prune) {
        const int padded = (p.njobs + 7) & ~7;
        qb = lin / padded;
        job = lin % padded;
    }
    if (job >= p.njobs) return;

    int b, sub;
    if (MODE == MODE_SCORE) {
        b = job / p.subCount;
        sub = p.subBegin + job % p.subCount;
        job = b * 12 + sub;
    }
    else if (MODE == MODE_NN) { b = job; sub = 0; }
    else { b = job >> 1; sub = job & 1; }

    CloudView qc, tc;
    PointXf qxf, txf;
    qxf.kind = XF_NONE; txf.kind = XF_NONE;
    qxf.a = affine_identity(); txf.a = qxf.a;

    if (MODE == MODE_NN) {
        qc.base = p.A + (size_t)b * p.N * p.strideQ; qc.stride = p.strideQ;
        qc.n = p.lenA ? p.lenA[b] : p.N;
        tc.base = p.C + (size_t)b * p.NT * p.strideT; tc.stride = p.strideT;
        tc.n = p.lenC ? p.lenC[b] : p.NT;
    } else {
        const bool sw = p.swap != nullptr && p.swap[b] != 0;
        CloudView a, c;
        a.base = (sw ? p.C : p.A) + (size_t)b * p.N * 4; a.stride = 4; a.n = (sw ? p.lenC : p.lenA)[b];
        c.base = (sw ? p.A : p.C) + (size_t)b * p.N * 4; c.stride = 4; c.n = (sw ? p.lenA : p.lenC)[b];
        PointXf axf;
        axf.a = affine_identity();
        if (MODE == MODE_SCORE) {
            const int k = sub >> 1;
            axf.kind = XF_TRANSLATE;
            const float *t = p.cand + ((size_t)b * 6 + k) * 3;
            axf.a.t[0] = t[0]; axf.a.t[1] = t[1]; axf.a.t[2] = t[2];
        } else if (MODE == MODE_CHECK) {
            axf.kind = XF_AFFINE;
            axf.a = affine_from_pose((sub == 0 ? p.poseA : p.poseB) + (size_t)b * 16);
        } else {
            axf.kind = XF_AFFINE;
            axf.a = affine_from_pose(p.poseA + (size_t)b * 16);
// ... 881 lines not shown
                                        int qblocks, int32_t *__restrict__ tab)
{
    const int k = blockIdx.x * blockDim.x + threadIdx.x;
    if (k >= B) return;
    const int b = pairOrder != nullptr ? pairOrder[k] : k;
    const bool sw = swap != nullptr && swap[b] != 0;
    const int na = (sw ? lenC : lenA)[b], nc = (sw ? lenA : lenC)[b];
    const int nqs[4] = {na, nc, lenA[b], lenC[b]}, nts[4] = {nc, na, lenC[b], lenA[b]};
#pragma unroll
    for (int d = 0; d < 4; ++d) {
        const int nq = nqs[d], nt = nts[d];
        const int nqb = (nq + kSweepBlock - 1) / kSweepBlock;
        const bool fullScan = nq > 0 && nqb <= kSweepFullQb && nt >= kSweepFullScanMinNt && qblocks >= 2 * nqb;
        const int shares = fullScan ? min(qblocks / nqb, kSweepShares) : 1;
        tab[k * 4 + d] = (b << 16) | (min(shares * nqb, 255) << 8) | min(nqb, 255);
    }
}

hipError_t launch_sweep_pair_table(const int32_t *lenA, const int32_t *lenC, const uint8_t *swap, const int32_t *pairOrder,
                                   int B, int N, int32_t *tab, hipStream_t s)
{
    if (B > 32767 || sweep_qblocks(N) > 255) return hipErrorInvalidValue;
    hipLaunchKernelGGL(sweep_pair_table_kernel, dim3((B + 255) / 256), dim3(256), 0, s, lenA, lenC, swap, pairOrder, B,
                       sweep_qblocks(N), tab);
    return hipGetLastError();
}

template <int MODE>
static hipError_t launch_sweep(SweepParams p, hipStream_t s)
{
    p.NP16 = (p.N + kChunk - 1) / kChunk * kChunk;
    p.qblocks = sweep_qblocks(p.N);
    p.r0 = 0.15f;
#ifndef ICPFLOW_NO_SWEEP_SHARE
    p.shareWindows = 1;
#endif
#ifdef ICPFLOW_NO_SWEEP_SHARE
    p.shareCount = nullptr;
#endif
    if (p.N < kSweepFullScanMinTargets || p.shareBest == nullptr) p.shareCount = nullptr;
    if (p.shareCount != nullptr && !p.shareClean) {
        const hipError_t me = hipMemsetAsync(p.shareCount, 0, (size_t)(MODE == SWEEP_SCORE ? (p.njobs / p.subCount) * 12 : p.njobs) * kSweepFullQb * sizeof(int), s);
        if (me != hipSuccess) return me;
    }
    const int groups = (MODE == SWEEP_CHECK && p.initSum != nullptr) ? 2 * ((p.njobs / 2 + 7) / 8) : (p.njobs + 7) / 8;
    const size_t lds = (size_t)((p.NP16 < kSweepStage ? p.NP16 : kSweepStage) * 33 / 32 + 1) * sizeof(float);
    const int total = groups * 8 * p.qblocks;
    if (MODE == SWEEP_SCORE && p.listMode == 1) {
        const int first = groups * 8;
        if (p.shareWindows != 0 && p.N >= kSweepFullScanMinTargets && p.njobs <= 12 * 700)
            hipLaunchKernelGGL((sweep_scan_kernel<MODE, true>), dim3((unsigned)first), dim3(kSweepBlock), lds, s, p);
        else
            hipLaunchKernelGGL((sweep_scan_kernel<MODE, false>), dim3((unsigned)first), dim3(kSweepBlock), lds, s, p);
        return hipGetLastError();
    }
    if (MODE == SWEEP_SCORE && p.listMode == 2) {
        const int wgs = total < 8 * 256 ? total : 8 * 256;
        if (p.shareWindows != 0 && p.N >= kSweepFullScanMinTargets && p.njobs <= 12 * 700)
            hipLaunchKernelGGL((sweep_list_kernel<MODE, true>), dim3((unsigned)wgs), dim3(kSweepBlock), lds, s, p);
        else
            hipLaunchKernelGGL((sweep_list_kernel<MODE, false>), dim3((unsigned)wgs), dim3(kSweepBlock), lds, s, p);
        return hipGetLastError();
    }
    if (MODE == SWEEP_SCORE && p.pairSlots > 0) {
        const unsigned blocks = (unsigned)((p.njobs / p.subCount) * (p.qblocks * p.pairSlots + 10 - p.pairSlots));
        if (p.shareWindows != 0 && p.N >= kSweepFullScanMinTargets && p.njobs <= 12 * 700)
            hipLaunchKernelGGL((sweep_pair_kernel<true>), dim3(blocks), dim3(kSweepBlock), lds, s, p);
        else
            hipLaunchKernelGGL((sweep_pair_kernel<false>), dim3(blocks), dim3(kSweepBlock), lds, s, p);
        return hipGetLastError();
    }
    unsigned blocks = (unsigned)total;
    if (MODE == SWEEP_SCORE && p.totBase != 0) {
        p.totBase = total;
        blocks += (unsigned)((p.njobs / p.subCount) * 10);
    }
    if (p.shareWindows != 0 && p.N >= kSweepFullScanMinTargets && p.njobs <= 12 * 700)
        hipLaunchKernelGGL((sweep_scan_kernel<MODE, true>), dim3(blocks), dim3(kSweepBlock), lds, s, p);
    else
        hipLaunchKernelGGL((sweep_scan_kernel<MODE, false>), dim3(blocks), dim3(kSweepBlock), lds, s, p);
    return hipGetLastError();
}

constexpr int kOccBlock = 256;
__device__ __forceinline__ uint32_t occ_shifted(const uint32_t *in, int w, int sh, bool up)
{
    const int q = sh >> 5, r = sh & 31;
    if (up) {
        const int a = w - q;
        const uint32_t lo = a >= 0 ? in[a] : 0u, lo1 = a - 1 >= 0 ? in[a - 1] : 0u;
        return r == 0 ? lo : ((lo << r) | (lo1 >> (32 - r)));
    }
    const int a = w + q;
    const uint32_t hi = a < kOccWords ? in[a] : 0u, hi1 = a + 1 < kOccWords ? in[a + 1] : 0u;
    return r == 0 ? hi : ((hi >> r) | (hi1 << (32 - r)));
}

template <bool RAW>
__global__ __launch_bounds__(kOccBlock) void occ_build_kernel(const float *__restrict__ Xsoa, const float *__restrict__ Ysoa,
                                                            int NP16, float *__restrict__ hdrOut, uint32_t *__restrict__ bitsOut,
                                                            const int32_t *__restrict__ lenX, const int32_t *__restrict__ lenY,
                                                            const uint8_t *__restrict__ swap, int selfCount)
{
    __shared__ uint32_t bitsA[kOccWords], bitsB[kOccWords];
    __shared__ float red[6 * (kOccBlock / kWave)];
    __shared__ float hd[8];
    const int b = blockIdx.x, which = blockIdx.y, tid = threadIdx.x, lane = tid & (kWave - 1), wave = tid >> 6;
    const float *px, *py, *pz;
    int rows = NP16;
    constexpr int kStep = RAW ? 4 : 1;
    if (RAW) {
        int cX, cY;
        bool sw;
        if (selfCount) {
            __shared__ int cntScratch[2 * (kOccBlock / kWave)];
            const float4 *qx = reinterpret_cast<const float4 *>(Xsoa) + (size_t)b * NP16;
            const float4 *qy = reinterpret_cast<const float4 *>(Ysoa) + (size_t)b * NP16;
            int c[2] = {0, 0};
            for (int i = tid; i < NP16; i += kOccBlock) {
                c[0] += (qx[i].w > 0.0f) ? 1 : 0;
                c[1] += (qy[i].w > 0.0f) ? 1 : 0;
            }
            block_sum<2, int>(c, cntScratch);
            cX = c[0]; cY = c[1];
            sw = selfCount == 2 && cX > cY;
        } else {
            cX = lenX[b]; cY = lenY[b];
            sw = swap != nullptr && swap[b] != 0;
        }
        const bool fromY = (which == 0) == sw;
        px = (fromY ? Ysoa : Xsoa) + (size_t)b * NP16 * 4; py = px + 1; pz = px + 2;
        rows = fromY ? cY : cX;
    } else {
        px = (which == 0 ? Xsoa : Ysoa) + (size_t)b * 3 * NP16; py = px + NP16; pz = py + NP16;
    }
    for (int k = tid; k < kOccWords; k += kOccBlock) bitsA[k] = 0u;
    float mn[3] = {kInf, kInf, kInf}, mx[3] = {-kInf, -kInf, -kInf};
    for (int i = tid; i < rows; i += kOccBlock) {
        const float x = px[i * kStep], y = py[i * kStep], z = pz[i * kStep];
        if (fabsf(x) < 1e30f && fabsf(y) < 1e30f && fabsf(z) < 1e30f) {
            mn[0] = fminf(mn[0], x); mn[1] = fminf(mn[1], y); mn[2] = fminf(mn[2], z);
            mx[0] = fmaxf(mx[0], x); mx[1] = fmaxf(mx[1], y); mx[2] = fmaxf(mx[2], z);
        }
    }
#pragma unroll
    for (int a = 0; a < 3; ++a) {
#pragma unroll
        for (int o = kWave / 2; o > 0; o >>= 1) {
            mn[a] = fminf(mn[a], __shfl_xor(mn[a], o, kWave));
            mx[a] = fmaxf(mx[a], __shfl_xor(mx[a], o, kWave));
        }
        if (lane == 0) { red[wave * 6 + a] = mn[a]; red[wave * 6 + 3 + a] = mx[a]; }
    }
    __syncthreads();
    if (tid == 0) {
        float lo[3], hi[3];
        for (int a = 0; a < 3; ++a) {
            lo[a] = kInf; hi[a] = -kInf;
            for (int w = 0; w < kOccBlock / kWave; ++w) { lo[a] = fminf(lo[a], red[w * 6 + a]); hi[a] = fmaxf(hi[a], red[w * 6 + 3 + a]); }
        }
        int n[3] = {0, 0, 0};
        float h = 0.125f;
        if (lo[0] <= hi[0]) {
            for (int grow = 0; grow < 64; ++grow) {
                bool fits = true;
                long long cells = 1;
                for (int a = 0; a < 3; ++a) {
                    const float e = (hi[a] - lo[a]) / h;
                    if (!(e < 30000.f)) { fits = false; break; }
                    n[a] = (int)e + 2 + 2 * kOccRings;
                    cells *= n[a];
                }
                if (fits && cells <= (long long)kOccWords * 32) break;
                h *= 1.25f; n[0] = 0;
            }
        }
        if (n[0] <= 0) n[0] = n[1] = n[2] = 0;
        hd[0] = lo[0] - kOccRings * h; hd[1] = lo[1] - kOccRings * h; hd[2] = lo[2] - kOccRings * h;
        float big = 0.f;
        for (int a = 0; a < 3; ++a) big = fmaxf(big, fmaxf(fabsf(lo[a]), fabsf(hi[a])));
        if (!(big * 2.4e-7f / h < 0.005f)) n[0] = n[1] = n[2] = 0;
        hd[3] = 1.0f / h; hd[4] = 0.98f * h;
        hd[5] = __int_as_float(n[0]); hd[6] = __int_as_float(n[1]); hd[7] = __int_as_float(n[2]);
    }
    __syncthreads();
    const float gox = hd[0], goy = hd[1], goz = hd[2], ginv = hd[3];
    const int gnx = __float_as_int(hd[5]), gny = __float_as_int(hd[6]), gnz = __float_as_int(hd[7]);
    if (gnx > 0) {
        for (int i = tid; i < rows; i += kOccBlock) {
            const float x = px[i * kStep], y = py[i * kStep], z = pz[i * kStep];
            if (!(fabsf(x) < 1e30f && fabsf(y) < 1e30f && fabsf(z) < 1e30f)) continue;
            const int cx = min(max((int)floorf((x - gox) * ginv), kOccRings), gnx - 1 - kOccRings);
            const int cy = min(max((int)floorf((y - goy) * ginv), kOccRings), gny - 1 - kOccRings);
            const int cz = min(max((int)floorf((z - goz) * ginv), kOccRings), gnz - 1 - kOccRings);
            const int c = (cx * gny + cy) * gnz + cz;
            atomicOr(&bitsA[c >> 5], 1u << (c & 31));
        }
    }
    __syncthreads();
    const int strides[3] = {1, gnz, gny * gnz};
    uint32_t *in = bitsA, *outb = bitsB;
    uint32_t *bo = bitsOut + ((size_t)b * 2 + which) * kOccRings * kOccWords;
    for (int ring = 0; ring < kOccRings; ++ring) {
        for (int a = 0; a < 3; ++a) {
            if (gnx > 0)
                for (int w = tid; w < kOccWords; w += kOccBlock) outb[w] = in[w] | occ_shifted(in, w, strides[a], true) | occ_shifted(in, w, strides[a], false);
            __syncthreads();
            uint32_t *t = in; in = outb; outb = t;
        }
        for (int k = tid; k < kOccWords; k += kOccBlock) bo[ring * kOccWords + k] = gnx > 0 ? in[k] : 0u;
    }
    if (tid < 8) hdrOut[((size_t)b * 2 + which) * 8 + tid] = hd[tid];
}

hipError_t launch_occupancy(const GridScratch *grid, int B, int N, hipStream_t s)
{
    if (grid->occHdr == nullptr || grid->occBits == nullptr || grid->sortXsoa == nullptr || grid->sortYsoa == nullptr) return hipSuccess;
    const int NP16 = (N + kChunk - 1) / kChunk * kChunk;
    hipLaunchKernelGGL(occ_build_kernel<false>, dim3(B, 2), dim3(kOccBlock), 0, s, grid->sortXsoa, grid->sortYsoa, NP16, grid->occHdr, grid->occBits,
                       (const int32_t *)nullptr, (const int32_t *)nullptr, (const uint8_t *)nullptr, 0);
    return hipGetLastError();
}

hipError_t launch_occupancy_raw(const float *X, const float *Y, const int32_t *lenX, const int32_t *lenY, const uint8_t *swap, int B, int N,
                                const GridScratch *grid, int selfCount, hipStream_t s)
{
    if (grid->occHdr == nullptr || grid->occBits == nullptr || grid->sortXsoa == nullptr || grid->sortYsoa == nullptr) return hipSuccess;
    hipLaunchKernelGGL(occ_build_kernel<true>, dim3(B, 2), dim3(kOccBlock), 0, s, X, Y, N, grid->occHdr, grid->occBits, lenX, lenY, swap, selfCount);
    return hipGetLastError();
}

hipError_t launch_sweep_score(const GridScratch *grid, const int32_t *lenA, const int32_t *lenC, const uint8_t *swap,
                              int B, int N, const float *cand, double *partial, hipStream_t s)
{
    SweepParams p{};
    p.Asoa = grid->sortXsoa; p.Csoa = grid->sortYsoa; p.lenA = lenA; p.lenC = lenC; p.swap = swap;
    p.axis = grid->axis; p.cand = cand; p.N = N; p.njobs = B * 12; p.partial = partial;
    p.subBegin = 0; p.subCount = 12;
    p.shareBest = grid->shareBest; p.shareCount = grid->shareCount; p.shareClean = grid->shareCountClean; p.pairOrder = grid->pairOrder; p.pairTab = grid->pairTab;
    return launch_sweep<SWEEP_SCORE>(p, s);
}

hipError_t launch_sweep_score_pruned(const GridScratch *grid, const int32_t *lenA, const int32_t *lenC,
                                     const uint8_t *swap, int B, int N, const float *cand, double *partial,
                                     double *accum, hipStream_t s)
{
    SweepParams p{};
    p.Asoa = grid->sortXsoa; p.Csoa = grid->sortYsoa; p.lenA = lenA; p.lenC = lenC; p.swap = swap;
    p.axis = grid->axis; p.cand = cand; p.N = N; p.partial = partial; p.accum = accum;
    if (grid->occReady) { p.occHdr = grid->occHdr; p.occBits = grid->occBits; }
    p.shareBest = grid->shareBest; p.shareCount = grid->shareCount; p.shareClean = grid->shareCountClean; p.pairOrder = grid->pairOrder; p.pairTab = grid->pairTab;
    if (grid->occReady) {
#ifndef ICPFLOW_SCORE_LIST_MIN_JOBS
#define ICPFLOW_SCORE_LIST_MIN_JOBS 65536
#endif
        const bool listed = grid->sweepTicket != nullptr && grid->scoreList != nullptr &&
                            (long long)B * 10 * sweep_qblocks(N) >= ICPFLOW_SCORE_LIST_MIN_JOBS;
#ifndef ICPFLOW_SCORE_PAIR_MAX_BLOCKS
#define ICPFLOW_SCORE_PAIR_MAX_BLOCKS 1024
#endif
#ifndef ICPFLOW_SCORE_PAIR_WHOLE_MAX_QBLOCKS
#define ICPFLOW_SCORE_PAIR_WHOLE_MAX_QBLOCKS 4
#endif
        const bool byPair = kSweepPairSlots > 0 && !listed && grid->occTot != nullptr && (long long)B * sweep_qblocks(N) <= ICPFLOW_SCORE_PAIR_MAX_BLOCKS;
        p.njobs = B * 2; p.subBegin = 0; p.subCount = 2; p.prune = 0;
        if (byPair) { p.occTot = grid->occTot; p.totBase = 1; }
        hipError_t e2 = launch_sweep<SWEEP_SCORE>(p, s);
        if (e2 != hipSuccess) return e2;
        p.totBase = 0;
        p.njobs = B * 10; p.subBegin = 2; p.subCount = 10; p.prune = 1; p.boundBoth = 1;
        if (byPair) {
            p.pairSlots = sweep_qblocks(N) <= ICPFLOW_SCORE_PAIR_WHOLE_MAX_QBLOCKS ? kSweepPairSlots : 10;
            return launch_sweep<SWEEP_SCORE>(p, s);
        }
        if (listed) {
            p.list = grid->scoreList; p.listCount = grid->sweepTicket;
            p.listMode = 1;
            const hipError_t e3 = launch_sweep<SWEEP_SCORE>(p, s);
            if (e3 != hipSuccess) return e3;
            p.listMode = 2;
        }
        return launch_sweep<SWEEP_SCORE>(p, s);
    }
    p.njobs = B; p.subBegin = 0; p.subCount = 1; p.prune = 0;
    hipError_t e = launch_sweep<SWEEP_SCORE>(p, s);
    if (e != hipSuccess) return e;
    p.njobs = B * 11; p.subBegin = 1; p.subCount = 11; p.prune = 1;
    return launch_sweep<SWEEP_SCORE>(p, s);
}

hipError_t launch_sweep_eval(const GridScratch *grid, const int32_t *len1, const int32_t *len2, int B, int N,
                             const float *pose, float thres, float *srcT, double *partial, hipStream_t s,
                             const uint8_t *swap, const uint8_t *active)
{
    SweepParams p{};
// ... 122 lines not shown
```

### include/icpflow_hip.h

```cpp
#ifndef ICPFLOW_HIP_H
#define ICPFLOW_HIP_H

#include <stddef.h>
#include <stdint.h>

#ifdef __cplusplus
extern "C" {
#endif

#define ICPFLOW_VERSION 214

#define ICPFLOW_OK 0
#define ICPFLOW_E_ARG (-1)
#define ICPFLOW_E_WORKSPACE (-2)
#define ICPFLOW_E_LIMIT (-3)
#define ICPFLOW_E_HOSTMEM (-4)

#define ICPFLOW_STOP_REFERENCE 0
#define ICPFLOW_STOP_PER_PAIR 1

typedef void *icpflow_stream_t;

int icpflow_version(void);
const char *icpflow_last_error(void);
const char *icpflow_build_info(void);

#define ICPFLOW_SEARCH_AUTO 0
#define ICPFLOW_SEARCH_SCAN 1
#define ICPFLOW_SEARCH_GRID 2
#define ICPFLOW_SEARCH_SWEEP 3
#define ICPFLOW_ARITH_FP64 0
#define ICPFLOW_ARITH_FP32_REFERENCE 1
#define ICPFLOW_OPT_NO_SORTED_VOTE (1u << 0)
#define ICPFLOW_OPT_NO_SIDE_STREAM (1u << 1)
#define ICPFLOW_OPT_NO_EVAL_SWEEP (1u << 2)
#define ICPFLOW_OPT_NO_CHECK_SWEEP (1u << 3)
#define ICPFLOW_OPT_NO_SCORE_SWEEP (1u << 4)
#define ICPFLOW_OPT_NO_SCORE_PRUNE (1u << 5)
#define ICPFLOW_OPT_NO_TEAMS (1u << 6)
#define ICPFLOW_OPT_NO_SPECULATIVE (1u << 7)
#define ICPFLOW_OPT_NO_ADAPTIVE_WINDOWS (1u << 8)
#define ICPFLOW_OPT_NO_PERSISTENT (1u << 9)
#define ICPFLOW_OPT_NO_HELPERS (1u << 10)
#define ICPFLOW_OPT_TEAMS_HALF_GPU (1u << 11)
#define ICPFLOW_OPT_NO_SHARED_SCANS (1u << 12)
#define ICPFLOW_OPT_NO_STAGE_OVERLAP (1u << 13)
#define ICPFLOW_OPT_NO_VOTE_LIST (1u << 14)
#define ICPFLOW_OPT_NO_CHECK_REUSE (1u << 15)
#define ICPFLOW_OPT_NO_SCORE_PREBOUND (1u << 16)
#define ICPFLOW_OPT_TWO_LAUNCH (1u << 17)
#define ICPFLOW_OPT_NO_DIR_KEYS (1u << 18)

typedef struct icpflow_profile icpflow_profile_t;

typedef struct icpflow_options {
    size_t struct_size;
    int icp_search;
    int icp_arith;
    unsigned flags;
    icpflow_profile_t *profile;
    uint32_t *d_vote_bins_u32;
    const float *d_icp_init_R;
    const float *d_icp_init_T;
    float *d_icp_history;
    int icp_allow_reflection;
    int icp_estimate_scale;
    float *d_icp_scale;
    const float *d_icp_init_s;
    const uint8_t *d_pair_active;
} icpflow_options_t;

size_t icpflow_workspace_bytes(int B, int N, int Lx, int Ly, int Lz);

int icpflow_hist_vote(const float *d_X, const float *d_Y, int B, int NX, int NY,
                      float min_x, float min_y, float min_z,
                      float max_x, float max_y, float max_z,
                      int len_x, int len_y, int len_z,
                      float *d_bins, icpflow_stream_t stream);

int icpflow_hist_peaks(const float *d_bins, int B, int len_x, int len_y, int len_z,
                       int k, int kernel_size, float *d_votes, int64_t *d_idx,
                       void *d_ws, size_t ws_bytes, icpflow_stream_t stream);

int icpflow_nn_batch(const float *d_Q, const float *d_T, int B, int NQ, int NT,
                     int q_stride, int t_stride, const int32_t *d_len_q,
                     const int32_t *d_len_t, int sqrt_dist, int64_t *d_idx,
                     float *d_dist, icpflow_stream_t stream);

int icpflow_transform_points(const float *d_xyz, const float *d_pose, int B, int N,
                             float *d_out, icpflow_stream_t stream);

int icpflow_count_valid(const float *d_pts, int B, int N, int32_t *d_len,
                        icpflow_stream_t stream);

int icpflow_estimate_init_pose(const float *d_src, const float *d_dst, int B, int N,
                               const float *d_edges_x, int len_x,
                               const float *d_edges_y, int len_y,
                               const float *d_edges_z, int len_z,
                               float decode_shift, float *d_T_out,
                               void *d_ws, size_t ws_bytes, icpflow_stream_t stream,
                               const icpflow_options_t *opt);

int icpflow_icp(const float *d_X, const float *d_Y, const float *d_pre_pose, int B, int N,
                double thres, int max_iterations, double relative_rmse_thr, int stop_mode,
                float *d_R, float *d_T, float *d_rmse, int32_t *d_iters,
                int32_t *d_converged, void *d_ws, size_t ws_bytes,
                icpflow_stream_t stream, const icpflow_options_t *opt);

int icpflow_apply_icp(const float *d_src, const float *d_dst, const float *d_init,
                      int B, int N, double thres_dist, int max_iterations,
                      double relative_rmse_thr, int stop_mode, float *d_T_out,
                      int32_t *d_iters, void *d_ws, size_t ws_bytes,
                      icpflow_stream_t stream, const icpflow_options_t *opt);

int icpflow_hist_icp(const float *d_src, const float *d_dst, int B, int N,
                     const float *d_edges_x, int len_x,
                     const float *d_edges_y, int len_y,
                     const float *d_edges_z, int len_z,
                     float decode_shift, double thres_dist, int max_iterations,
                     double relative_rmse_thr, int stop_mode, float *d_T_out,
                     int32_t *d_iters, void *d_ws, size_t ws_bytes,
                     icpflow_stream_t stream, const icpflow_options_t *opt);

int icpflow_hist_icp_many(int K, const float *const *d_src, const float *const *d_dst, const int *B, int N,
                          const float *d_edges_x, int len_x, const float *d_edges_y, int len_y,
                          const float *d_edges_z, int len_z, float decode_shift, double thres_dist,
                          int max_iterations, double relative_rmse_thr, int stop_mode, float *const *d_T_out,
                          int32_t *const *d_iters, void *const *d_ws, const size_t *ws_bytes,
                          icpflow_stream_t stream, const icpflow_options_t *opt);

int icpflow_match_eval(const float *d_pcd1, const float *d_pcd2, const float *d_T,
                       int B, int N, double thres_dist, float *d_errors,
                       float *d_inliers, float *d_ratios, float *d_ious,
                       float *d_translations, float *d_rotations, void *d_ws,
// ... 301 lines not shown
```

Baseline: 419,600.

## Fuse cloud sorting and occupancy build into vote kernel as extra block roles

```diff
diff --git a/icp_flow_amd/_lib.py b/icp_flow_amd/_lib.py
--- a/icp_flow_amd/_lib.py
+++ b/icp_flow_amd/_lib.py
@@ -139,6 +139,9 @@
              "no_stage_overlap": 1 << 13, "no_vote_list": 1 << 14, "no_check_reuse": 1 << 15, "no_score_prebound": 1 << 16,
              "two_launch": 1 << 17,
              "no_dir_keys": 1 << 18}
+OPT_FLAGS_214 = {
+    "no_front_roles": 1 << 19}
+_ALL_FLAGS = {**OPT_FLAGS, **OPT_FLAGS_214}
 
 
 class Options(ctypes.Structure):
@@ -279,7 +282,7 @@
 
 def _env_default_flags():
     f = 0
-    for name, bit in OPT_FLAGS.items():
+    for name, bit in _ALL_FLAGS.items():
         if os.environ.get("ICPFLOW_" + name.upper(), "0") not in ("0", ""):
             f |= bit
     return f
@@ -318,7 +321,7 @@
     if pair_active is not None:
         cur["pair_active"] = pair_active
     for k, v in switches.items():
-        cur["flags"] = (cur["flags"] | OPT_FLAGS[k]) if v else (cur["flags"] & ~OPT_FLAGS[k])
+        cur["flags"] = (cur["flags"] | _ALL_FLAGS[k]) if v else (cur["flags"] & ~_ALL_FLAGS[k])
     stack = getattr(_tls, "stack", None)
     if stack is None:
         stack = _tls.stack = []
diff --git a/icp_flow_amd/build.py b/icp_flow_amd/build.py
--- a/icp_flow_amd/build.py
+++ b/icp_flow_amd/build.py
@@ -11,7 +11,7 @@
 OUT = os.path.join(HERE, "libicpflow_hip.so")
 SOURCES = ["api.hip", "hist.hip", "nn.hip", "icp.hip", "icp_prep.hip", "icp_plan.hip", "icp_epilogue.hip", "device.hip", "icp_fp32.hip", "pose.hip", "sort.hip", "cluster.hip", "hdbscan.hip", "clusterpcd.hip", "table.hip", "assoc.hip", "frame.hip", "ego.hip", "seqeval.hip", "classeval.hip", "bucketeval.hip", "segeval.hip", "ground.hip",
            "hdbscan_tree.cpp"]
-HEADERS = ["common.hpp", "scan.hpp", "kernels.hpp", "kabsch.hpp", "posefuse.hpp", "votekey.hpp", "cluster_util.hpp", "sortdir.hpp", "host.hpp", "carver.hpp", "rowerr.hpp", "clusterpcd_host.hpp", "gridhash.hpp", "icp_instr.hip",
+HEADERS = ["common.hpp", "scan.hpp", "kernels.hpp", "kabsch.hpp", "posefuse.hpp", "votekey.hpp", "cluster_util.hpp", "sortdir.hpp", "sortclouds.hpp", "occgrid.hpp", "host.hpp", "carver.hpp", "rowerr.hpp", "clusterpcd_host.hpp", "gridhash.hpp", "icp_instr.hip",
            os.path.join("..", "..", "include", "icpflow_hip.h")]
 CFLAGS = ["--offload-arch=gfx950", "-O3", "-std=c++17", "-fPIC", "-ffp-contract=off",
           "-fhip-fp32-correctly-rounded-divide-sqrt", "-Wall", "-Wno-unused-function"]
diff --git a/icp_flow_amd/csrc/api.hip b/icp_flow_amd/csrc/api.hip
--- a/icp_flow_amd/csrc/api.hip
+++ b/icp_flow_amd/csrc/api.hip
@@ -251,7 +251,7 @@
         return report_errorf(ICPFLOW_E_ARG, "%s: options.icp_search must be 0..3 (got %d)", fn, opt->icp_search);
     if (opt->icp_arith != ICPFLOW_ARITH_FP64 && opt->icp_arith != ICPFLOW_ARITH_FP32_REFERENCE)
         return report_errorf(ICPFLOW_E_ARG, "%s: options.icp_arith must be 0 or 1 (got %d)", fn, opt->icp_arith);
-    if (opt->flags >> 19) return report_errorf(ICPFLOW_E_ARG, "%s: unknown option flags 0x%x", fn, opt->flags);
+    if (opt->flags >> 20) return report_errorf(ICPFLOW_E_ARG, "%s: unknown option flags 0x%x", fn, opt->flags);
     o.search = opt->icp_search;
     o.arith = opt->icp_arith;
     o.flags = opt->flags;
@@ -422,7 +422,7 @@
 int run_init_pose(const float *src, const float *dst, Workspace &w, const uint8_t *swap, int B,
                   int N, const float *ex, int lx, const float *ey, int ly, const float *ez, int lz,
                   float shift, float *Tout, const Opts &o, hipStream_t s, hipEvent_t joinBefore = nullptr,
-                  const PairCountFuse *countFuse = nullptr, bool sideBusy = false)
+                  const PairCountFuse *countFuse = nullptr, bool sideBusy = false, const FrontRoles *roles = nullptr)
 {
     const int lens[3] = {lx, ly, lz};
     if (N <= kMaxSortN && o.on(ICPFLOW_OPT_NO_SORTED_VOTE)) {
@@ -430,7 +430,7 @@
         ICPFLOW_TRY(launch_hist_vote_sorted(dst, src, w.lenC, w.lenA, B, N, lens, ex, ey, ez, swap, w.zsortC,
                                             w.zsortA, w.bins, w.zckey, w.zcidx, w.voteKey, s, countFuse, sideBusy,
                                             w.grid.pairBox, o.on(ICPFLOW_OPT_NO_VOTE_LIST) ? w.voteWork : nullptr, w.voteWorkCap,
-                                            w.pairOrder, &planned));
+                                            w.pairOrder, &planned, roles));
         if (planned) w.grid.pairOrder = w.pairOrder;
     } else
         ICPFLOW_TRY(launch_hist_vote(dst, src, B, N, N, nullptr, nullptr, lens, ex, ey, ez, swap, w.bins, s));
@@ -1019,7 +1019,16 @@
     JoinGuard guard;
     const GridScratch *search = search_scratch(w, N, o);
     SideStream *side = nullptr;
-    if (search != nullptr && search->mode == 3 && N >= 64 && o.on(ICPFLOW_OPT_NO_SIDE_STREAM)) {
+    const int lens[3] = {len_x, len_y, len_z};
+    const bool sideWanted = search != nullptr && search->mode == 3 && N >= 64 && o.on(ICPFLOW_OPT_NO_SIDE_STREAM);
+    const bool frontRoles = sideWanted && countInSort && o.on(ICPFLOW_OPT_NO_FRONT_ROLES) && vote_front_roles_fit(B, N, lens);
+    FrontRoles roles{};
+    if (frontRoles) {
+        roles.src = d_src; roles.dst = d_dst; roles.lenSrc = w.lenA; roles.lenDst = w.lenC; roles.grid = &w.grid;
+        roles.occ = score_by_sweep(N, true, o) && o.on(ICPFLOW_OPT_NO_SCORE_PRUNE) && o.on(ICPFLOW_OPT_NO_SCORE_PREBOUND);
+        w.grid.presorted = 1;
+        if (roles.occ) w.grid.occReady = 1;
+    } else if (sideWanted) {
         side = &side_stream(s);
         if (!side->ok) side = nullptr;
     }
@@ -1059,10 +1068,10 @@
     }
     w.grid.shareCountClean = 1;
     w.grid.sweepTicket = w.ticketScratch;
-    const bool sweepScore = score_by_sweep(N, join != nullptr, o);
+    const bool sweepScore = score_by_sweep(N, join != nullptr || frontRoles, o);
     if (int r = run_init_pose(d_src, d_dst, w, w.swap, B, N, d_edges_x, len_x, d_edges_y, len_y, d_edges_z,
                               len_z, decode_shift, w.Tinit, o, s, sweepScore ? join : nullptr,
-                              countInSort ? &fuse : nullptr, join != nullptr))
+                              countInSort ? &fuse : nullptr, join != nullptr, frontRoles ? &roles : nullptr))
         return r;
     if (join != nullptr && !sweepScore) ICPFLOW_TRY(hipStreamWaitEvent(s, join, 0));
     guard.joined();
diff --git a/icp_flow_amd/csrc/hist.hip b/icp_flow_amd/csrc/hist.hip
--- a/icp_flow_amd/csrc/hist.hip
+++ b/icp_flow_amd/csrc/hist.hip
@@ -1,6 +1,8 @@
 #include "common.hpp"
 #include "kernels.hpp"
 #include "votekey.hpp"
+#include "sortclouds.hpp"
+#include "occgrid.hpp"
 
 namespace icpflow {
 
@@ -370,23 +372,23 @@
     }
 }
 
-template <int BLOCK, int SPLIT = 1>
-__global__ __launch_bounds__(BLOCK) void hist_vote_sorted_kernel(
+template <int BLOCK, int SPLIT>
+__device__ __forceinline__ void hist_vote_sorted_body(
+    unsigned char *smem, int bx, int by,
     const float4 *__restrict__ Xs, const float4 *__restrict__ Ys, const int32_t *__restrict__ nXv,
     const int32_t *__restrict__ nYv, int N, int len_x, int len_y, int len_z,
     const float *__restrict__ ex, const float *__restrict__ ey, const float *__restrict__ ez,
     const uint8_t *__restrict__ swap, int useLds, uint32_t *__restrict__ bins_u32,
     const float *__restrict__ keyRec, int span, const int32_t *__restrict__ work, int nPairs)
 {
-    extern __shared__ __attribute__((aligned(16))) unsigned char smem[];
     float4 *tile = reinterpret_cast<float4 *>(smem);
     uint32_t *lhist = reinterpret_cast<uint32_t *>(smem + sizeof(float4) * kVoteTile);
     int item = 0;
     if (work != nullptr) {
-        item = work[blockIdx.x];
+        item = work[bx];
         if (item < 0) return;
     }
-    const int b = work != nullptr ? (item & 1023) : (int)blockIdx.y;
+    const int b = work != nullptr ? (item & 1023) : by;
     const VoteKey vk = vote_key_load(keyRec + (size_t)b * kVoteKeyStride);
     const bool sw = swap != nullptr && swap[b] != 0;
     const float4 *xb = (sw ? Ys : Xs) + (size_t)b * N;
@@ -396,8 +398,8 @@
     constexpr int kRows = BLOCK / SPLIT;
     constexpr int kRowWaves = kRows / kWave;
     const int rowBlocks = work != nullptr ? (nx + kRows - 1) / kRows : (N + kRows - 1) / kRows;
-    const int rb = work != nullptr ? ((item >> 10) & 255) : (int)blockIdx.x / tsplit;
-    const int jBegin = (work != nullptr ? (item >> 18) : (int)blockIdx.x % tsplit) * span;
+    const int rb = work != nullptr ? ((item >> 10) & 255) : bx / tsplit;
+    const int jBegin = (work != nullptr ? (item >> 18) : bx % tsplit) * span;
     if (rb * kWave >= nx || jBegin >= ny) return;
     const float min_x = ex[0], max_x = ex[len_x - 1];
     const float min_y = ey[0], max_y = ey[len_y - 1];
@@ -505,6 +507,19 @@
     }
 }
 
+template <int BLOCK, int SPLIT = 1>
+__global__ __launch_bounds__(BLOCK) void hist_vote_sorted_kernel(
+    const float4 *__restrict__ Xs, const float4 *__restrict__ Ys, const int32_t *__restrict__ nXv,
+    const int32_t *__restrict__ nYv, int N, int len_x, int len_y, int len_z,
+    const float *__restrict__ ex, const float *__restrict__ ey, const float *__restrict__ ez,
+    const uint8_t *__restrict__ swap, int useLds, uint32_t *__restrict__ bins_u32,
+    const float *__restrict__ keyRec, int span, const int32_t *__restrict__ work, int nPairs)
+{
+    extern __shared__ __attribute__((aligned(16))) unsigned char smem[];
+    hist_vote_sorted_body<BLOCK, SPLIT>(smem, (int)blockIdx.x, (int)blockIdx.y, Xs, Ys, nXv, nYv, N, len_x, len_y, len_z, ex, ey, ez,
+                                        swap, useLds, bins_u32, keyRec, span, work, nPairs);
+}
+
 __global__ __launch_bounds__(1024) void vote_plan_kernel(const int32_t *__restrict__ nXv, const int32_t *__restrict__ nYv,
                                                          const uint8_t *__restrict__ swap, int nPairs, int rows, int span,
                                                          int U, int32_t *__restrict__ work, int32_t *__restrict__ orderOut)
@@ -551,6 +566,82 @@
     work[e] = item;
 }
 
+#ifndef ICPFLOW_VOTE_WIDE_N
+#define ICPFLOW_VOTE_WIDE_N 1023
+#endif
+#ifndef ICPFLOW_VOTE_LIST_MIN_N
+#define ICPFLOW_VOTE_LIST_MIN_N 4097
+#endif
+#ifndef ICPFLOW_VOTE_LIST_SPAN
+#define ICPFLOW_VOTE_LIST_SPAN 2048
+#endif
+#ifndef ICPFLOW_VOTE_WIDE_B
+#define ICPFLOW_VOTE_WIDE_B 2
+#endif
+constexpr int kVoteListSpan = ICPFLOW_VOTE_LIST_SPAN;
+constexpr int kVoteWideB = ICPFLOW_VOTE_WIDE_B;
+constexpr int kVoteWideN = ICPFLOW_VOTE_WIDE_N;
+
+struct FrontRoleArgs {
+    const float *X, *Y;
+    const int32_t *lenX, *lenY;
+    int32_t *axisOut;
+    float4 *Xs, *Ys;
+    float *Ysoa, *Xsoa;
+    float *occHdr;
+    uint32_t *occBits;
+    int NP2, dirKeys, nOcc, nSort, rows;
+};
+constexpr int kFrontBlock = 512;
+
+__global__ __launch_bounds__(kFrontBlock) void front_roles_kernel(
+    const float4 *__restrict__ Xs, const float4 *__restrict__ Ys, const int32_t *__restrict__ nXv,
+    const int32_t *__restrict__ nYv, int N, int len_x, int len_y, int len_z,
+    const float *__restrict__ ex, const float *__restrict__ ey, const float *__restrict__ ez,
+    const uint8_t *__restrict__ swap, int useLds, uint32_t *__restrict__ bins_u32,
+    const float *__restrict__ keyRec, int span, int nPairs, FrontRoleArgs r)
+{
+    extern __shared__ __attribute__((aligned(16))) unsigned char smem[];
+    if ((int)blockIdx.y < r.rows) {
+        const int id = (int)(blockIdx.y * gridDim.x + blockIdx.x);
+        if (id < r.nOcc) {
+            const int which = (int)threadIdx.x / kOccBlock;
+            uint32_t *bits = reinterpret_cast<uint32_t *>(smem + which * kOccLdsBytes);
+            float *red = reinterpret_cast<float *>(bits + 2 * kOccWords);
+            const OccLds lds{bits, bits + kOccWords, red, red + 6 * (kOccBlock / kWave), nullptr};
+            occ_build_body<true>(lds, id, which, (int)threadIdx.x % kOccBlock, r.X, r.Y, N, r.occHdr, r.occBits, r.lenX, r.lenY, swap, 0);
+        } else if (id < r.nOcc + r.nSort) {
+            const int job = id - r.nOcc;
+            unsigned long long *kv = reinterpret_cast<unsigned long long *>(smem);
+            float *bb = reinterpret_cast<float *>(kv + r.NP2);
+            float *box = bb + 6 * (kFrontBlock / kWave);
+            int *axis = reinterpret_cast<int *>(box + 6);
+            const SortLds lds{kv, bb, box, axis, reinterpret_cast<unsigned int *>(axis + 1), nullptr};
+            sort_clouds_body<kFrontBlock>(lds, job >> 1, (job & 1) != 0, (int)threadIdx.x, r.X, r.Y, r.lenX, r.lenY, swap, nullptr, N,
+                                          r.NP2, r.axisOut, r.Xs, r.Ys, r.Ysoa, r.Xsoa, 0, r.dirKeys);
+        }
+        return;
+    }
+    hist_vote_sorted_body<kFrontBlock, 4>(smem, (int)blockIdx.x, (int)blockIdx.y - r.rows, Xs, Ys, nXv, nYv, N, len_x, len_y, len_z, ex,
+                                          ey, ez, swap, useLds, bins_u32, keyRec, span, nullptr, nPairs);
+}
+
+static size_t vote_lds_bytes(const int lens[3])
+{
+    const size_t L = (size_t)lens[0] * lens[1] * lens[2];
+    return sizeof(float4) * kVoteTile + sizeof(uint32_t) * (L + (size_t)vote_overflow_bins(lens[1], lens[2]));
+}
+
+bool vote_front_roles_fit(int B, int N, const int lens[3])
+{
+    const size_t lds = vote_lds_bytes(lens);
+    if (lds > 64 * 1024 || N <= kVoteWideN || N > kChunkSortMinN || N >= ICPFLOW_VOTE_LIST_MIN_N || B > kVoteWideB * device_cus())
+        return false;
+    int NP2 = 64;
+    while (NP2 < N) NP2 <<= 1;
+    return (size_t)NP2 * 8 + (size_t)sort_lds_small_bytes(kFrontBlock) <= lds && 2 * (size_t)kOccLdsBytes <= lds;
+}
+
 size_t vote_work_capacity(int B, int N)
 {
     if (N <= 1023 || B > 1024) return 0;
@@ -563,9 +654,10 @@
                                    const float *ez, const uint8_t *swap, float *sortX, float *sortY,
                                    uint32_t *bins_u32, float *ckey, int *cidx, float *keyRec, hipStream_t s,
                                    const PairCountFuse *fuse, bool sideBusy, const float *boxes, int32_t *work, size_t workCap,
-                                   int32_t *orderOut, bool *planned)
+                                   int32_t *orderOut, bool *planned, const FrontRoles *roles)
 {
     if (planned != nullptr) *planned = false;
+    if (roles != nullptr && !vote_front_roles_fit(B, N, lens)) return hipErrorInvalidValue;
     if (fuse != nullptr && N > kChunkSortMinN) return hipErrorInvalidValue;
     const size_t L = (size_t)lens[0] * lens[1] * lens[2];
     int NP2 = 64;
@@ -592,21 +684,6 @@
     const size_t tile_bytes = sizeof(float4) * kVoteTile;
     const size_t lds_hist = tile_bytes + sizeof(uint32_t) * (L + (size_t)vote_overflow_bins(lens[1], lens[2]));
     const int useLds = lds_hist <= 64 * 1024;
-#ifndef ICPFLOW_VOTE_WIDE_N
-#define ICPFLOW_VOTE_WIDE_N 1023
-#endif
-#ifndef ICPFLOW_VOTE_LIST_MIN_N
-#define ICPFLOW_VOTE_LIST_MIN_N 4097
-#endif
-#ifndef ICPFLOW_VOTE_LIST_SPAN
-#define ICPFLOW_VOTE_LIST_SPAN 2048
-#endif
-    constexpr int kVoteListSpan = ICPFLOW_VOTE_LIST_SPAN;
-#ifndef ICPFLOW_VOTE_WIDE_B
-#define ICPFLOW_VOTE_WIDE_B 2
-#endif
-    constexpr int kVoteWideB = ICPFLOW_VOTE_WIDE_B;
-    constexpr int kVoteWideN = ICPFLOW_VOTE_WIDE_N;
     const int cus = device_cus();
     const long long wgs256 = (long long)((N + kVoteBlock - 1) / kVoteBlock) * ((N + kVoteSpan * kVoteTile - 1) / (kVoteSpan * kVoteTile)) * B;
     int block = wgs256 >= 4LL * cus ? 512 : kVoteBlock;
@@ -630,6 +707,20 @@
                                (int)U, work, orderOut);
             if (planned != nullptr) *planned = orderOut != nullptr;
             grid = dim3((unsigned)U, 1);
+        }
+        if (roles != nullptr) {
+            const GridScratch *g = roles->grid;
+            const bool occ = roles->occ && g->occHdr != nullptr && g->occBits != nullptr && g->sortXsoa != nullptr && g->sortYsoa != nullptr;
+            FrontRoleArgs r{};
+            r.X = roles->src; r.Y = roles->dst; r.lenX = roles->lenSrc; r.lenY = roles->lenDst;
+            r.axisOut = g->axis; r.Xs = (float4 *)g->sortX; r.Ys = (float4 *)g->pts; r.Ysoa = g->sortYsoa; r.Xsoa = g->sortXsoa;
+            r.occHdr = g->occHdr; r.occBits = g->occBits;
+            r.NP2 = NP2; r.dirKeys = g->dirKeys; r.nOcc = occ ? B : 0; r.nSort = 2 * B;
+            r.rows = (r.nOcc + r.nSort + (int)grid.x - 1) / (int)grid.x;
+            hipLaunchKernelGGL(front_roles_kernel, dim3(grid.x, (unsigned)(r.rows + B)), dim3(kFrontBlock), lds_hist, s,
+                               (const float4 *)sortX, (const float4 *)sortY, nX, nY, N, lens[0], lens[1], lens[2], ex, ey,
+                               ez, swap, useLds, bins_u32, keyRec, span, B, r);
+            return hipGetLastError();
         }
         hipLaunchKernelGGL((hist_vote_sorted_kernel<512, 4>), grid, dim3(512), lds_hist, s,
                            (const float4 *)sortX, (const float4 *)sortY, nX, nY, N, lens[0], lens[1], lens[2], ex, ey,
diff --git a/icp_flow_amd/csrc/icp_prep.hip b/icp_flow_amd/csrc/icp_prep.hip
--- a/icp_flow_amd/csrc/icp_prep.hip
+++ b/icp_flow_amd/csrc/icp_prep.hip
@@ -1,5 +1,6 @@
 #include "scan.hpp"
 #include "sortdir.hpp"
+#include "sortclouds.hpp"
 #include "kernels.hpp"
 #include "gridhash.hpp"
 
@@ -83,104 +84,14 @@
     float *__restrict__ Ysoa, float *__restrict__ Xsoa, int selfCount, int dirKeys)
 {
     extern __shared__ __attribute__((aligned(16))) unsigned char dynLds[];
-    unsigned long long *kv = reinterpret_cast<unsigned long long *>(dynLds);
     __shared__ float bb[6 * (kSortBlock / kWave)];
+    __shared__ float boxSh[6];
     __shared__ int axisSh;
-    const int b = blockIdx.x, tid = threadIdx.x;
-    const bool moving = blockIdx.y == 1;
-    int cX, cY;
-    bool sw;
-    if (selfCount) {
-        __shared__ int cntScratch[2 * (kSortBlock / kWave)];
-        const float4 *px = reinterpret_cast<const float4 *>(X) + (size_t)b * N;
-        const float4 *py = reinterpret_cast<const float4 *>(Y) + (size_t)b * N;
-        int c[2] = {0, 0};
-        for (int i = tid; i < N; i += kSortBlock) {
-            c[0] += (px[i].w > 0.0f) ? 1 : 0;
-            c[1] += (py[i].w > 0.0f) ? 1 : 0;
-        }
-        block_sum<2, int>(c, cntScratch);
-        cX = c[0]; cY = c[1];
-        sw = selfCount == 2 && cX > cY;
-    } else {
-        cX = lenX[b]; cY = lenY[b];
-        sw = swap != nullptr && swap[b] != 0;
-    }
-    const float4 *xb = reinterpret_cast<const float4 *>(sw ? Y : X) + (size_t)b * N;
-    const float4 *yb = reinterpret_cast<const float4 *>(sw ? X : Y) + (size_t)b * N;
-    const int nx = sw ? cY : cX, ny = sw ? cX : cY;
-    float mn[3] = {kInf, kInf, kInf}, mx[3] = {-kInf, -kInf, -kInf};
-    for (int j = tid; j < ny; j += kSortBlock) {
-        const float4 q = yb[j];
-        mn[0] = fminf(mn[0], q.x); mn[1] = fminf(mn[1], q.y); mn[2] = fminf(mn[2], q.z);
-        mx[0] = fmaxf(mx[0], q.x); mx[1] = fmaxf(mx[1], q.y); mx[2] = fmaxf(mx[2], q.z);
-    }
-#pragma unroll
-    for (int k = 0; k < 3; ++k)
-#pragma unroll
-        for (int o = kWave / 2; o > 0; o >>= 1) {
-            mn[k] = fminf(mn[k], __shfl_xor(mn[k], o, kWave));
-            mx[k] = fmaxf(mx[k], __shfl_xor(mx[k], o, kWave));
-        }
-    if ((tid & (kWave - 1)) == 0) {
-#pragma unroll
-        for (int k = 0; k < 3; ++k) { bb[(tid >> 6) * 6 + k] = mn[k]; bb[(tid >> 6) * 6 + 3 + k] = mx[k]; }
-    }
-    __syncthreads();
-    __shared__ float boxSh[6];
-    if (tid == 0) {
-        float e[3];
-        for (int k = 0; k < 3; ++k) {
-            float lo = bb[k], hi = bb[3 + k];
-            for (int w = 1; w < kSortBlock / kWave; ++w) { lo = fminf(lo, bb[w * 6 + k]); hi = fmaxf(hi, bb[w * 6 + 3 + k]); }
-            e[k] = hi - lo;
-            boxSh[k] = lo; boxSh[3 + k] = hi;
-        }
-        const int a = (e[0] >= e[1] && e[0] >= e[2]) ? 0 : (e[1] >= e[2] ? 1 : 2);
-        axisSh = a;
-    }
-    __syncthreads();
-    if (dirKeys && ny >= kSortDirMinN && nx >= kSortDirMinMoving) {
-        __shared__ unsigned int scoreSh[kSortCodes];
-        (void)choose_sort_code<kSortBlock>(yb, ny, boxSh, axisSh, reinterpret_cast<unsigned int *>(dynLds), scoreSh, &axisSh);
-    }
-    if (tid == 0 && !moving) axisOut[b] = axisSh;
-    const int axis = axisSh;
-    float dirX = 0.f, dirY = 0.f;
-    if (axis >= 3) sort_dir(axis, dirX, dirY);
-    const int n = moving ? nx : ny;
-    const float4 *cloud = moving ? xb : yb;
-    PointXf pre;
-    pre.kind = (moving && prePose) ? XF_AFFINE : XF_NONE;
-    pre.a = (moving && prePose) ? affine_from_pose(prePose + (size_t)b * 16) : affine_identity();
-    int np2 = kWave;
-    while (np2 < n) np2 <<= 1;
-    np2 = min(np2, NP2);
-    for (int j = tid; j < np2; j += kSortBlock) {
-        float k = kInf;
-        if (j < n) {
-            const float4 q = cloud[j];
-            float px, py, pz;
-            xf_apply(pre, q.x, q.y, q.z, px, py, pz);
-            k = sort_key_of(axis, dirX, dirY, px, py, pz);
-        }
-        kv[j] = sort_pack(k, j);
-    }
-    __syncthreads();
-    bitonic_sort_lds(kv, np2);
-    float4 *out = (moving ? Xs : Ys) + (size_t)b * N;
-    const int NP16 = (N + kChunk - 1) / kChunk * kChunk;
-    float *soa = moving ? (Xsoa ? Xsoa + (size_t)b * 3 * NP16 : nullptr) : Ysoa + (size_t)b * 3 * NP16;
-    for (int r = tid; r < (soa ? NP16 : n); r += kSortBlock) {
-        float px = kInf, py = kInf, pz = kInf;
-        if (r < n) {
-            const int j = sort_index_of(kv[r]);
-            const float4 q = cloud[j];
-            xf_apply(pre, q.x, q.y, q.z, px, py, pz);
-            out[r] = make_float4(px, py, pz, __int_as_float(j));
-        }
-        if (soa) { soa[r] = px; soa[NP16 + r] = py; soa[2 * NP16 + r] = pz; }
-    }
+    __shared__ unsigned int scoreSh[kSortCodes];
+    __shared__ int cntScratch[2 * (kSortBlock / kWave)];
+    const SortLds lds{reinterpret_cast<unsigned long long *>(dynLds), bb, boxSh, &axisSh, scoreSh, cntScratch};
+    sort_clouds_body<kSortBlock>(lds, blockIdx.x, blockIdx.y == 1, threadIdx.x, X, Y, lenX, lenY, swap, prePose, N, NP2, axisOut, Xs,
+                                 Ys, Ysoa, Xsoa, selfCount, dirKeys);
 }
 
 static bool sort_is_chunked(int N, const GridScratch *grid) { return N > kChunkSortMinN && grid->ckey != nullptr; }
diff --git a/icp_flow_amd/csrc/kernels.hpp b/icp_flow_amd/csrc/kernels.hpp
--- a/icp_flow_amd/csrc/kernels.hpp
+++ b/icp_flow_amd/csrc/kernels.hpp
@@ -105,12 +105,21 @@
     void *zero0; size_t bytes0;
     void *zero1; size_t bytes1;
 };
+struct GridScratch;
+struct FrontRoles {
+    const float *src, *dst;
+    const int32_t *lenSrc, *lenDst;
+    const GridScratch *grid;
+    bool occ;
+};
+bool vote_front_roles_fit(int B, int N, const int lens[3]);
 hipError_t launch_hist_vote_sorted(const float *X, const float *Y, int32_t *nX, int32_t *nY,
                                    int B, int N, const int lens[3], const float *ex, const float *ey,
                                    const float *ez, const uint8_t *swap, float *sortX, float *sortY,
                                    uint32_t *bins_u32, float *ckey, int *cidx, float *keyRec, hipStream_t s,
                                    const PairCountFuse *fuse = nullptr, bool sideBusy = false, const float *boxes = nullptr,
-                                   int32_t *work = nullptr, size_t workCap = 0, int32_t *orderOut = nullptr, bool *planned = nullptr);
+                                   int32_t *work = nullptr, size_t workCap = 0, int32_t *orderOut = nullptr, bool *planned = nullptr,
+                                   const FrontRoles *roles = nullptr);
 size_t vote_work_capacity(int B, int N);
 constexpr int kChunkSortMinN = 4096;
 constexpr int kPairBoxStride = 24;
diff --git a/icp_flow_amd/csrc/nn.hip b/icp_flow_amd/csrc/nn.hip
--- a/icp_flow_amd/csrc/nn.hip
+++ b/icp_flow_amd/csrc/nn.hip
@@ -2,6 +2,7 @@
 #include "sortdir.hpp"
 #include "kernels.hpp"
 #include "posefuse.hpp"
+#include "occgrid.hpp"
 
 namespace icpflow {
 
@@ -1049,20 +1050,6 @@
     return hipGetLastError();
 }
 
-constexpr int kOccBlock = 256;
-__device__ __forceinline__ uint32_t occ_shifted(const uint32_t *in, int w, int sh, bool up)
-{
-    const int q = sh >> 5, r = sh & 31;
-    if (up) {
-        const int a = w - q;
-        const uint32_t lo = a >= 0 ? in[a] : 0u, lo1 = a - 1 >= 0 ? in[a - 1] : 0u;
-        return r == 0 ? lo : ((lo << r) | (lo1 >> (32 - r)));
-    }
-    const int a = w + q;
-    const uint32_t hi = a < kOccWords ? in[a] : 0u, hi1 = a + 1 < kOccWords ? in[a + 1] : 0u;
-    return r == 0 ? hi : ((hi >> r) | (hi1 << (32 - r)));
-}
-
 template <bool RAW>
 __global__ __launch_bounds__(kOccBlock) void occ_build_kernel(const float *__restrict__ Xsoa, const float *__restrict__ Ysoa,
                                                             int NP16, float *__restrict__ hdrOut, uint32_t *__restrict__ bitsOut,
@@ -1072,112 +1059,9 @@
     __shared__ uint32_t bitsA[kOccWords], bitsB[kOccWords];
     __shared__ float red[6 * (kOccBlock / kWave)];
     __shared__ float hd[8];
-    const int b = blockIdx.x, which = blockIdx.y, tid = threadIdx.x, lane = tid & (kWave - 1), wave = tid >> 6;
-    const float *px, *py, *pz;
-    int rows = NP16;
-    constexpr int kStep = RAW ? 4 : 1;
-    if (RAW) {
-        int cX, cY;
-        bool sw;
-        if (selfCount) {
-            __shared__ int cntScratch[2 * (kOccBlock / kWave)];
-            const float4 *qx = reinterpret_cast<const float4 *>(Xsoa) + (size_t)b * NP16;
-            const float4 *qy = reinterpret_cast<const float4 *>(Ysoa) + (size_t)b * NP16;
-            int c[2] = {0, 0};
-            for (int i = tid; i < NP16; i += kOccBlock) {
-                c[0] += (qx[i].w > 0.0f) ? 1 : 0;
-                c[1] += (qy[i].w > 0.0f) ? 1 : 0;
-            }
-            block_sum<2, int>(c, cntScratch);
-            cX = c[0]; cY = c[1];
-            sw = selfCount == 2 && cX > cY;
-        } else {
-            cX = lenX[b]; cY = lenY[b];
-            sw = swap != nullptr && swap[b] != 0;
-        }
-        const bool fromY = (which == 0) == sw;
-        px = (fromY ? Ysoa : Xsoa) + (size_t)b * NP16 * 4; py = px + 1; pz = px + 2;
-        rows = fromY ? cY : cX;
-    } else {
-        px = (which == 0 ? Xsoa : Ysoa) + (size_t)b * 3 * NP16; py = px + NP16; pz = py + NP16;
-    }
-    for (int k = tid; k < kOccWords; k += kOccBlock) bitsA[k] = 0u;
-    float mn[3] = {kInf, kInf, kInf}, mx[3] = {-kInf, -kInf, -kInf};
-    for (int i = tid; i < rows; i += kOccBlock) {
-        const float x = px[i * kStep], y = py[i * kStep], z = pz[i * kStep];
-        if (fabsf(x) < 1e30f && fabsf(y) < 1e30f && fabsf(z) < 1e30f) {
-            mn[0] = fminf(mn[0], x); mn[1] = fminf(mn[1], y); mn[2] = fminf(mn[2], z);
-            mx[0] = fmaxf(mx[0], x); mx[1] = fmaxf(mx[1], y); mx[2] = fmaxf(mx[2], z);
-        }
-    }
-#pragma unroll
-    for (int a = 0; a < 3; ++a) {
-#pragma unroll
-        for (int o = kWave / 2; o > 0; o >>= 1) {
-            mn[a] = fminf(mn[a], __shfl_xor(mn[a], o, kWave));
-            mx[a] = fmaxf(mx[a], __shfl_xor(mx[a], o, kWave));
-        }
-        if (lane == 0) { red[wave * 6 + a] = mn[a]; red[wave * 6 + 3 + a] = mx[a]; }
-    }
-    __syncthreads();
-    if (tid == 0) {
-        float lo[3], hi[3];
-        for (int a = 0; a < 3; ++a) {
-            lo[a] = kInf; hi[a] = -kInf;
-            for (int w = 0; w < kOccBlock / kWave; ++w) { lo[a] = fminf(lo[a], red[w * 6 + a]); hi[a] = fmaxf(hi[a], red[w * 6 + 3 + a]); }
-        }
-        int n[3] = {0, 0, 0};
-        float h = 0.125f;
-        if (lo[0] <= hi[0]) {
-            for (int grow = 0; grow < 64; ++grow) {
-                bool fits = true;
-                long long cells = 1;
-                for (int a = 0; a < 3; ++a) {
-                    const float e = (hi[a] - lo[a]) / h;
-                    if (!(e < 30000.f)) { fits = false; break; }
-                    n[a] = (int)e + 2 + 2 * kOccRings;
-                    cells *= n[a];
-                }
-                if (fits && cells <= (long long)kOccWords * 32) break;
-                h *= 1.25f; n[0] = 0;
-            }
-        }
-        if (n[0] <= 0) n[0] = n[1] = n[2] = 0;
-        hd[0] = lo[0] - kOccRings * h; hd[1] = lo[1] - kOccRings * h; hd[2] = lo[2] - kOccRings * h;
-        float big = 0.f;
-        for (int a = 0; a < 3; ++a) big = fmaxf(big, fmaxf(fabsf(lo[a]), fabsf(hi[a])));
-        if (!(big * 2.4e-7f / h < 0.005f)) n[0] = n[1] = n[2] = 0;
-        hd[3] = 1.0f / h; hd[4] = 0.98f * h;
-        hd[5] = __int_as_float(n[0]); hd[6] = __int_as_float(n[1]); hd[7] = __int_as_float(n[2]);
-    }
-    __syncthreads();
-    const float gox = hd[0], goy = hd[1], goz = hd[2], ginv = hd[3];
-    const int gnx = __float_as_int(hd[5]), gny = __float_as_int(hd[6]), gnz = __float_as_int(hd[7]);
-    if (gnx > 0) {
-        for (int i = tid; i < rows; i += kOccBlock) {
-            const float x = px[i * kStep], y = py[i * kStep], z = pz[i * kStep];
-            if (!(fabsf(x) < 1e30f && fabsf(y) < 1e30f && fabsf(z) < 1e30f)) continue;
-            const int cx = min(max((int)floorf((x - gox) * ginv), kOccRings), gnx - 1 - kOccRings);
-            const int cy = min(max((int)floorf((y - goy) * ginv), kOccRings), gny - 1 - kOccRings);
-            const int cz = min(max((int)floorf((z - goz) * ginv), kOccRings), gnz - 1 - kOccRings);
-            const int c = (cx * gny + cy) * gnz + cz;
-            atomicOr(&bitsA[c >> 5], 1u << (c & 31));
-        }
-    }
-    __syncthreads();
-    const int strides[3] = {1, gnz, gny * gnz};
-    uint32_t *in = bitsA, *outb = bitsB;
-    uint32_t *bo = bitsOut + ((size_t)b * 2 + which) * kOccRings * kOccWords;
-    for (int ring = 0; ring < kOccRings; ++ring) {
-        for (int a = 0; a < 3; ++a) {
-            if (gnx > 0)
-                for (int w = tid; w < kOccWords; w += kOccBlock) outb[w] = in[w] | occ_shifted(in, w, strides[a], true) | occ_shifted(in, w, strides[a], false);
-            __syncthreads();
-            uint32_t *t = in; in = outb; outb = t;
-        }
-        for (int k = tid; k < kOccWords; k += kOccBlock) bo[ring * kOccWords + k] = gnx > 0 ? in[k] : 0u;
-    }
-    if (tid < 8) hdrOut[((size_t)b * 2 + which) * 8 + tid] = hd[tid];
+    __shared__ int cntScratch[2 * (kOccBlock / kWave)];
+    const OccLds lds{bitsA, bitsB, red, hd, cntScratch};
+    occ_build_body<RAW>(lds, blockIdx.x, blockIdx.y, threadIdx.x, Xsoa, Ysoa, NP16, hdrOut, bitsOut, lenX, lenY, swap, selfCount);
 }
 
 hipError_t launch_occupancy(const GridScratch *grid, int B, int N, hipStream_t s)
diff --git a/icp_flow_amd/csrc/occgrid.hpp b/icp_flow_amd/csrc/occgrid.hpp
--- /dev/null
+++ b/icp_flow_amd/csrc/occgrid.hpp
@@ -0,0 +1,145 @@
+#pragma once
+#include "common.hpp"
+#include "kernels.hpp"
+
+namespace icpflow {
+
+constexpr int kOccBlock = 256;
+__device__ __forceinline__ uint32_t occ_shifted(const uint32_t *in, int w, int sh, bool up)
+{
+    const int q = sh >> 5, r = sh & 31;
+    if (up) {
+        const int a = w - q;
+        const uint32_t lo = a >= 0 ? in[a] : 0u, lo1 = a - 1 >= 0 ? in[a - 1] : 0u;
+        return r == 0 ? lo : ((lo << r) | (lo1 >> (32 - r)));
+    }
+    const int a = w + q;
+    const uint32_t hi = a < kOccWords ? in[a] : 0u, hi1 = a + 1 < kOccWords ? in[a + 1] : 0u;
+    return r == 0 ? hi : ((hi >> r) | (hi1 << (32 - r)));
+}
+
+struct OccLds {
+    uint32_t *bitsA, *bitsB;
+    float *red;
+    float *hd;
+    int *cnt;
+};
+constexpr int kOccLdsBytes = 2 * kOccWords * 4 + (6 * (kOccBlock / kWave) + 8) * 4;
+
+template <bool RAW>
+__device__ __forceinline__ void occ_build_body(const OccLds &lds, int b, int which, int tid, const float *__restrict__ Xsoa,
+                                               const float *__restrict__ Ysoa, int NP16, float *__restrict__ hdrOut,
+                                               uint32_t *__restrict__ bitsOut, const int32_t *__restrict__ lenX,
+                                               const int32_t *__restrict__ lenY, const uint8_t *__restrict__ swap, int selfCount)
+{
+    uint32_t *const bitsA = lds.bitsA, *const bitsB = lds.bitsB;
+    float *const red = lds.red, *const hd = lds.hd;
+    const int lane = tid & (kWave - 1), wave = tid >> 6;
+    const float *px, *py, *pz;
+    int rows = NP16;
+    constexpr int kStep = RAW ? 4 : 1;
+    if (RAW) {
+        int cX, cY;
+        bool sw;
+        if (selfCount) {
+            int *const cntScratch = lds.cnt;
+            const float4 *qx = reinterpret_cast<const float4 *>(Xsoa) + (size_t)b * NP16;
+            const float4 *qy = reinterpret_cast<const float4 *>(Ysoa) + (size_t)b * NP16;
+            int c[2] = {0, 0};
+            for (int i = tid; i < NP16; i += kOccBlock) {
+                c[0] += (qx[i].w > 0.0f) ? 1 : 0;
+                c[1] += (qy[i].w > 0.0f) ? 1 : 0;
+            }
+            block_sum<2, int>(c, cntScratch);
+            cX = c[0]; cY = c[1];
+            sw = selfCount == 2 && cX > cY;
+        } else {
+            cX = lenX[b]; cY = lenY[b];
+            sw = swap != nullptr && swap[b] != 0;
+        }
+        const bool fromY = (which == 0) == sw;
+        px = (fromY ? Ysoa : Xsoa) + (size_t)b * NP16 * 4; py = px + 1; pz = px + 2;
+        rows = fromY ? cY : cX;
+    } else {
+        px = (which == 0 ? Xsoa : Ysoa) + (size_t)b * 3 * NP16; py = px + NP16; pz = py + NP16;
+    }
+    for (int k = tid; k < kOccWords; k += kOccBlock) bitsA[k] = 0u;
+    float mn[3] = {kInf, kInf, kInf}, mx[3] = {-kInf, -kInf, -kInf};
+    for (int i = tid; i < rows; i += kOccBlock) {
+        const float x = px[i * kStep], y = py[i * kStep], z = pz[i * kStep];
+        if (fabsf(x) < 1e30f && fabsf(y) < 1e30f && fabsf(z) < 1e30f) {
+            mn[0] = fminf(mn[0], x); mn[1] = fminf(mn[1], y); mn[2] = fminf(mn[2], z);
+            mx[0] = fmaxf(mx[0], x); mx[1] = fmaxf(mx[1], y); mx[2] = fmaxf(mx[2], z);
+        }
+    }
+#pragma unroll
+    for (int a = 0; a < 3; ++a) {
+#pragma unroll
+        for (int o = kWave / 2; o > 0; o >>= 1) {
+            mn[a] = fminf(mn[a], __shfl_xor(mn[a], o, kWave));
+            mx[a] = fmaxf(mx[a], __shfl_xor(mx[a], o, kWave));
+        }
+        if (lane == 0) { red[wave * 6 + a] = mn[a]; red[wave * 6 + 3 + a] = mx[a]; }
+    }
+    __syncthreads();
+    if (tid == 0) {
+        float lo[3], hi[3];
+        for (int a = 0; a < 3; ++a) {
+            lo[a] = kInf; hi[a] = -kInf;
+            for (int w = 0; w < kOccBlock / kWave; ++w) { lo[a] = fminf(lo[a], red[w * 6 + a]); hi[a] = fmaxf(hi[a], red[w * 6 + 3 + a]); }
+        }
+        int n[3] = {0, 0, 0};
+        float h = 0.125f;
+        if (lo[0] <= hi[0]) {
+            for (int grow = 0; grow < 64; ++grow) {
+                bool fits = true;
+                long long cells = 1;
+                for (int a = 0; a < 3; ++a) {
+                    const float e = (hi[a] - lo[a]) / h;
+                    if (!(e < 30000.f)) { fits = false; break; }
+                    n[a] = (int)e + 2 + 2 * kOccRings;
+                    cells *= n[a];
+                }
+                if (fits && cells <= (long long)kOccWords * 32) break;
+                h *= 1.25f; n[0] = 0;
+            }
+        }
+        if (n[0] <= 0) n[0] = n[1] = n[2] = 0;
+        hd[0] = lo[0] - kOccRings * h; hd[1] = lo[1] - kOccRings * h; hd[2] = lo[2] - kOccRings * h;
+        float big = 0.f;
+        for (int a = 0; a < 3; ++a) big = fmaxf(big, fmaxf(fabsf(lo[a]), fabsf(hi[a])));
+        if (!(big * 2.4e-7f / h < 0.005f)) n[0] = n[1] = n[2] = 0;
+        hd[3] = 1.0f / h; hd[4] = 0.98f * h;
+        hd[5] = __int_as_float(n[0]); hd[6] = __int_as_float(n[1]); hd[7] = __int_as_float(n[2]);
+    }
+    __syncthreads();
+    const float gox = hd[0], goy = hd[1], goz = hd[2], ginv = hd[3];
+    const int gnx = __float_as_int(hd[5]), gny = __float_as_int(hd[6]), gnz = __float_as_int(hd[7]);
+    if (gnx > 0) {
+        for (int i = tid; i < rows; i += kOccBlock) {
+            const float x = px[i * kStep], y = py[i * kStep], z = pz[i * kStep];
+            if (!(fabsf(x) < 1e30f && fabsf(y) < 1e30f && fabsf(z) < 1e30f)) continue;
+            const int cx = min(max((int)floorf((x - gox) * ginv), kOccRings), gnx - 1 - kOccRings);
+            const int cy = min(max((int)floorf((y - goy) * ginv), kOccRings), gny - 1 - kOccRings);
+            const int cz = min(max((int)floorf((z - goz) * ginv), kOccRings), gnz - 1 - kOccRings);
+            const int c = (cx * gny + cy) * gnz + cz;
+            atomicOr(&bitsA[c >> 5], 1u << (c & 31));
+        }
+    }
+    __syncthreads();
+    const int strides[3] = {1, gnz, gny * gnz};
+    uint32_t *in = bitsA, *outb = bitsB;
+    uint32_t *bo = bitsOut + ((size_t)b * 2 + which) * kOccRings * kOccWords;
+    for (int ring = 0; ring < kOccRings; ++ring) {
+        for (int a = 0; a < 3; ++a) {
+            if (gnx > 0)
+                for (int w = tid; w < kOccWords; w += kOccBlock) outb[w] = in[w] | occ_shifted(in, w, strides[a], true) | occ_shifted(in, w, strides[a], false);
+            __syncthreads();
+            uint32_t *t = in; in = outb; outb = t;
+        }
+        for (int k = tid; k < kOccWords; k += kOccBlock) bo[ring * kOccWords + k] = gnx > 0 ? in[k] : 0u;
+    }
+    if (tid < 8) hdrOut[((size_t)b * 2 + which) * 8 + tid] = hd[tid];
+}
+
+}
diff --git a/icp_flow_amd/csrc/sortclouds.hpp b/icp_flow_amd/csrc/sortclouds.hpp
--- /dev/null
+++ b/icp_flow_amd/csrc/sortclouds.hpp
@@ -0,0 +1,122 @@
+#pragma once
+#include "scan.hpp"
+#include "sortdir.hpp"
+
+namespace icpflow {
+
+struct SortLds {
+    unsigned long long *kv;
+    float *bb;
+    float *box;
+    int *axis;
+    unsigned int *score;
+    int *cnt;
+};
+constexpr int sort_lds_small_bytes(int block) { return (6 * (block / kWave) + 6 + 1 + kSortCodes) * 4; }
+
+template <int BLOCK>
+__device__ __forceinline__ void sort_clouds_body(
+    const SortLds &lds, int b, bool moving, int tid, const float *__restrict__ X, const float *__restrict__ Y,
+    const int32_t *__restrict__ lenX, const int32_t *__restrict__ lenY, const uint8_t *__restrict__ swap,
+    const float *__restrict__ prePose, int N, int NP2, int32_t *__restrict__ axisOut, float4 *__restrict__ Xs,
+    float4 *__restrict__ Ys, float *__restrict__ Ysoa, float *__restrict__ Xsoa, int selfCount, int dirKeys)
+{
+    unsigned long long *const kv = lds.kv;
+    float *const bb = lds.bb;
+    int &axisSh = *lds.axis;
+    int cX, cY;
+    bool sw;
+    if (selfCount) {
+        int *const cntScratch = lds.cnt;
+        const float4 *px = reinterpret_cast<const float4 *>(X) + (size_t)b * N;
+        const float4 *py = reinterpret_cast<const float4 *>(Y) + (size_t)b * N;
+        int c[2] = {0, 0};
+        for (int i = tid; i < N; i += BLOCK) {
+            c[0] += (px[i].w > 0.0f) ? 1 : 0;
+            c[1] += (py[i].w > 0.0f) ? 1 : 0;
+        }
+        block_sum<2, int>(c, cntScratch);
+        cX = c[0]; cY = c[1];
+        sw = selfCount == 2 && cX > cY;
+    } else {
+        cX = lenX[b]; cY = lenY[b];
+        sw = swap != nullptr && swap[b] != 0;
+    }
+    const float4 *xb = reinterpret_cast<const float4 *>(sw ? Y : X) + (size_t)b * N;
+    const float4 *yb = reinterpret_cast<const float4 *>(sw ? X : Y) + (size_t)b * N;
+    const int nx = sw ? cY : cX, ny = sw ? cX : cY;
+    float mn[3] = {kInf, kInf, kInf}, mx[3] = {-kInf, -kInf, -kInf};
+    for (int j = tid; j < ny; j += BLOCK) {
+        const float4 q = yb[j];
+        mn[0] = fminf(mn[0], q.x); mn[1] = fminf(mn[1], q.y); mn[2] = fminf(mn[2], q.z);
+        mx[0] = fmaxf(mx[0], q.x); mx[1] = fmaxf(mx[1], q.y); mx[2] = fmaxf(mx[2], q.z);
+    }
+#pragma unroll
+    for (int k = 0; k < 3; ++k)
+#pragma unroll
+        for (int o = kWave / 2; o > 0; o >>= 1) {
+            mn[k] = fminf(mn[k], __shfl_xor(mn[k], o, kWave));
+            mx[k] = fmaxf(mx[k], __shfl_xor(mx[k], o, kWave));
+        }
+    if ((tid & (kWave - 1)) == 0) {
+#pragma unroll
+        for (int k = 0; k < 3; ++k) { bb[(tid >> 6) * 6 + k] = mn[k]; bb[(tid >> 6) * 6 + 3 + k] = mx[k]; }
+    }
+    __syncthreads();
+    float *const boxSh = lds.box;
+    if (tid == 0) {
+        float e[3];
+        for (int k = 0; k < 3; ++k) {
+            float lo = bb[k], hi = bb[3 + k];
+            for (int w = 1; w < BLOCK / kWave; ++w) { lo = fminf(lo, bb[w * 6 + k]); hi = fmaxf(hi, bb[w * 6 + 3 + k]); }
+            e[k] = hi - lo;
+            boxSh[k] = lo; boxSh[3 + k] = hi;
+        }
+        const int a = (e[0] >= e[1] && e[0] >= e[2]) ? 0 : (e[1] >= e[2] ? 1 : 2);
+        axisSh = a;
+    }
+    __syncthreads();
+    if (dirKeys && ny >= kSortDirMinN && nx >= kSortDirMinMoving) {
+        unsigned int *const scoreSh = lds.score;
+        (void)choose_sort_code<BLOCK>(yb, ny, boxSh, axisSh, reinterpret_cast<unsigned int *>(kv), scoreSh, &axisSh);
+    }
+    if (tid == 0 && !moving) axisOut[b] = axisSh;
+    const int axis = axisSh;
+    float dirX = 0.f, dirY = 0.f;
+    if (axis >= 3) sort_dir(axis, dirX, dirY);
+    const int n = moving ? nx : ny;
+    const float4 *cloud = moving ? xb : yb;
+    PointXf pre;
+    pre.kind = (moving && prePose) ? XF_AFFINE : XF_NONE;
+    pre.a = (moving && prePose) ? affine_from_pose(prePose + (size_t)b * 16) : affine_identity();
+    int np2 = kWave;
+    while (np2 < n) np2 <<= 1;
+    np2 = min(np2, NP2);
+    for (int j = tid; j < np2; j += BLOCK) {
+        float k = kInf;
+        if (j < n) {
+            const float4 q = cloud[j];
+            float px, py, pz;
+            xf_apply(pre, q.x, q.y, q.z, px, py, pz);
+            k = sort_key_of(axis, dirX, dirY, px, py, pz);
+        }
+        kv[j] = sort_pack(k, j);
+    }
+    __syncthreads();
+    bitonic_sort_lds(kv, np2);
+    float4 *out = (moving ? Xs : Ys) + (size_t)b * N;
+    const int NP16 = (N + kChunk - 1) / kChunk * kChunk;
+    float *soa = moving ? (Xsoa ? Xsoa + (size_t)b * 3 * NP16 : nullptr) : Ysoa + (size_t)b * 3 * NP16;
+    for (int r = tid; r < (soa ? NP16 : n); r += BLOCK) {
+        float px = kInf, py = kInf, pz = kInf;
+        if (r < n) {
+            const int j = sort_index_of(kv[r]);
+            const float4 q = cloud[j];
+            xf_apply(pre, q.x, q.y, q.z, px, py, pz);
+            out[r] = make_float4(px, py, pz, __int_as_float(j));
+        }
+        if (soa) { soa[r] = px; soa[NP16 + r] = py; soa[2 * NP16 + r] = pz; }
+    }
+}
+
+}
diff --git a/include/icpflow_hip.h b/include/icpflow_hip.h
--- a/include/icpflow_hip.h
+++ b/include/icpflow_hip.h
@@ -50,6 +50,7 @@
 #define ICPFLOW_OPT_NO_SCORE_PREBOUND (1u << 16)
 #define ICPFLOW_OPT_TWO_LAUNCH (1u << 17)
 #define ICPFLOW_OPT_NO_DIR_KEYS (1u << 18)
+#define ICPFLOW_OPT_NO_FRONT_ROLES (1u << 19)
 
 typedef struct icpflow_profile icpflow_profile_t;
 
```

Measured after the change: 426,500, median of 6. 1.02x the previous value.
